# pigBond/olympics-mujoco

Hardware: AMD Instinct MI355X
Metric: env-steps/sec, 4096 UnitreeH1.walk envs per GPU, obs+reward+done+ctrl HIP kernel (higher is better)
Workload: dtype f64; 1 GPU; UnitreeH1.walk config-2: fused K1+K5 over one [T,N] block per step; T=400, envs_per_gpu=4096, launch_regime=[T,N] block per launch, io=qpos/qvel f64 + action f32 in; obs/reward/ctrl f32 + absorbing u8 out, parallelism=env-sharded x1, no data-path collective

## Files before the change

olympics-mujoco_amd/csrc/host_batcher.hip:

```cpp
#include <atomic>
#include <chrono>
#include <condition_variable>
#include <mutex>
#include <thread>
#include <vector>

#include "oly_common.h"

struct WorkerPool {
  std::vector<std::thread> threads;
  std::mutex mu;
  std::condition_variable cv_go;
  std::atomic<long> generation{0};
  std::atomic<int> pending{0};
  std::atomic<int> sleepers{0};
  std::atomic<bool> stop{false};
  static constexpr int kSpinUs = 200;

  static double now() {
    return std::chrono::duration<double>(std::chrono::steady_clock::now().time_since_epoch()).count();
  }
  static void relax() { __builtin_ia32_pause(); }

  template <class Job>
  void start(int n, Job job) {
    for (int id = 0; id < n; ++id)
      threads.emplace_back([this, job, id] {
        long seen = 0;
        for (;;) {
          const double t0 = now();
          int polls = 0;
          while (generation.load(std::memory_order_acquire) == seen && !stop.load(std::memory_order_acquire)) {
            relax();
            if ((++polls & 63) == 0 && (now() - t0) * 1e6 > kSpinUs) {
              std::unique_lock<std::mutex> lk(mu);
              sleepers.fetch_add(1);
              cv_go.wait(lk, [&] { return stop.load() || generation.load() != seen; });
              sleepers.fetch_sub(1);
            }
          }
          if (stop.load(std::memory_order_acquire)) return;
          seen = generation.load(std::memory_order_acquire);
          job(id);
          pending.fetch_sub(1, std::memory_order_release);
        }
      });
  }
  void run() {
    pending.store((int)threads.size(), std::memory_order_relaxed);
    generation.fetch_add(1);
    if (sleepers.load() > 0) {
      std::lock_guard<std::mutex> lk(mu);
      cv_go.notify_all();
    }
    int polls = 0;
    while (pending.load(std::memory_order_acquire) != 0) {
      relax();
      if ((++polls & 1023) == 0) std::this_thread::yield();
    }
  }
  void shutdown() {
    {
      std::lock_guard<std::mutex> lk(mu);
      stop.store(true, std::memory_order_release);
    }
    cv_go.notify_all();
    for (auto& t : threads) t.join();
    threads.clear();
  }
};

struct oly_batcher {
  oly_ctx* ctx;
  int N, nq, nv, nu, n_act, n_threads;
  double dt;
  oly_physics_fn fn;
  void* user;
  double *h_qpos, *h_qvel, *h_ctrl;
  double *d_qpos, *d_qvel, *d_ctrl, *d_prev;
  int mapped;
  double *m_qpos, *m_qvel, *m_ctrl;
  int W, C;
  oly_physics_contacts_fn cfn;
  void* cuser;
  unsigned char *h_con, *d_con;
  size_t con_bytes, off_g1, off_g2, off_f6;
  double* d_grf;
  uint8_t* d_over;
  std::atomic<int> overflow_env;
  int packed;
  double *h_grfw, *d_grfw;
  std::vector<std::vector<unsigned char>> scratch;
  WorkerPool pool;
  double timing[3];
};

namespace {

void kinematic_step(int, const double*, double* qpos, double* qvel, void* user) {
  const oly_batcher* b = static_cast<const oly_batcher*>(user);
  const int n = b->nq < b->nv ? b->nq : b->nv;
  for (int i = 0; i < n; ++i) qpos[i] += b->dt * qvel[i];
}

void pack_env(oly_batcher* b, int e, const oly_il_contacts& oc, double* out_base) {
  const oly_ctx* ctx = b->ctx;
  const int P = ctx->grf.n_pairs, K = 3 * P, C = b->C;
  for (int w = 0; w < b->W; ++w) {
    const int nc_raw = oc.ncon[(size_t)w * oc.ncon_stride];
    if (!out_base && nc_raw >= 0 && nc_raw <= C) continue;
    double* out = out_base ? out_base + ((size_t)w * b->N + e) * K : nullptr;
    if (out) for (int k = 0; k < K; ++k) out[k] = 0.0;
    const int nc = nc_raw < 0 ? 0 : (nc_raw > C ? C : nc_raw);
    const int32_t *g1 = oc.geom1 + (size_t)w * oc.geom_stride, *g2 = oc.geom2 + (size_t)w * oc.geom_stride;
    const double* f6 = oc.force6 + (size_t)w * oc.force_stride;
    bool over = nc_raw < 0;
    for (int p = 0; p < P; ++p) {
      bool found = false;
      for (int i = 0; i < nc; ++i) {
        const int a = g1[i], c2 = g2[i];
        const int ga = (a >= 0 && a < ctx->grf.ngeom) ? ctx->grf_group_host[a] : -1;
        const int gb = (c2 >= 0 && c2 < ctx->grf.ngeom) ? ctx->grf_group_host[c2] : -1;
        if (ga < 0 || gb < 0) continue;
        if ((ga == ctx->grf.pair_a[p] && gb == ctx->grf.pair_b[p]) || (ga == ctx->grf.pair_b[p] && gb == ctx->grf.pair_a[p])) {
          if (out) { const double* f = f6 + (size_t)i * 6; out[3 * p] = f[0]; out[3 * p + 1] = f[1]; out[3 * p + 2] = f[2]; }
          found = true;
          break;
        }
      }
      if (!found && nc_raw > C) over = true;
    }
    if (over) {
      int none = -1;
      b->overflow_env.compare_exchange_strong(none, e);
    }
  }
}

void run_range(oly_batcher* b, int lo, int hi, int id) {
  if (b->cfn && b->packed) {
    const size_t W = (size_t)b->W, C = (size_t)b->C;
    unsigned char* sc = b->scratch[id].data();
    int32_t* ncon = reinterpret_cast<int32_t*>(sc);
    const size_t off_g1 = (sizeof(int32_t) * W + 15) & ~(size_t)15;
    const size_t off_g2 = off_g1 + sizeof(int32_t) * W * C;
    const size_t off_f6 = (off_g2 + sizeof(int32_t) * W * C + 15) & ~(size_t)15;
    for (int e = lo; e < hi; ++e) {
      oly_il_contacts oc;
      oc.W = b->W; oc.C = b->C;
      oc.ncon = ncon; oc.ncon_stride = 1;
      oc.geom1 = reinterpret_cast<int32_t*>(sc + off_g1);
      oc.geom2 = reinterpret_cast<int32_t*>(sc + off_g2);
      oc.geom_stride = (long)C;
      oc.force6 = reinterpret_cast<double*>(sc + off_f6);
      oc.force_stride = (long)(C * 6);
      b->cfn(e, b->h_ctrl + (size_t)e * b->nu, b->h_qpos + (size_t)e * b->nq, b->h_qvel + (size_t)e * b->nv, &oc,
             b->cuser);
      pack_env(b, e, oc, b->h_grfw);
    }
    return;
  }
  if (b->cfn) {
    const size_t N = (size_t)b->N, C = (size_t)b->C;
    for (int e = lo; e < hi; ++e) {
      oly_il_contacts oc;
      oc.W = b->W; oc.C = b->C;
      oc.ncon = reinterpret_cast<int32_t*>(b->h_con) + e; oc.ncon_stride = (long)N;
      oc.geom1 = reinterpret_cast<int32_t*>(b->h_con + b->off_g1) + (size_t)e * C;
      oc.geom2 = reinterpret_cast<int32_t*>(b->h_con + b->off_g2) + (size_t)e * C;
      oc.geom_stride = (long)(N * C);
      oc.force6 = reinterpret_cast<double*>(b->h_con + b->off_f6) + (size_t)e * C * 6;
      oc.force_stride = (long)(N * C * 6);
      b->cfn(e, b->h_ctrl + (size_t)e * b->nu, b->h_qpos + (size_t)e * b->nq, b->h_qvel + (size_t)e * b->nv, &oc,
             b->cuser);
      pack_env(b, e, oc, nullptr);
    }
    return;
  }
  void* user = b->fn == kinematic_step ? static_cast<void*>(b) : b->user;
  for (int e = lo; e < hi; ++e)
    b->fn(e, b->h_ctrl + (size_t)e * b->nu, b->h_qpos + (size_t)e * b->nq, b->h_qvel + (size_t)e * b->nv, user);
}

void worker_main(oly_batcher* b, int id) {
  const int per = (b->N + b->n_threads - 1) / b->n_threads;
  const int lo = id * per, hi = lo + per < b->N ? lo + per : b->N;
  if (lo < hi) run_range(b, lo, hi, id);
}

double now_s() {
  return std::chrono::duration<double>(std::chrono::steady_clock::now().time_since_epoch()).count();
}

}

extern "C" int oly_batcher_create(oly_batcher** out, oly_ctx* ctx, int N, int n_threads, double dt,
                                  oly_physics_fn physics, void* user) {
  if (!out || !ctx) return OLY_EINVAL;
  *out = nullptr;
  if (!ctx->il_ok) OLY_FAIL(ctx, OLY_ENOTCONF, "oly_batcher_create before oly_il_configure");
  if (N <= 0 || n_threads < 0) OLY_FAIL(ctx, OLY_EINVAL, "oly_batcher_create: bad N or n_threads");
  OLY_HIP(ctx, hipSetDevice(ctx->device));
  oly_batcher* b = new (std::nothrow) oly_batcher();
  if (!b) return OLY_ENOMEM;
  const IlDev& h = ctx->il_host;
  b->ctx = ctx; b->N = N; b->nq = h.nq; b->nv = h.nv; b->nu = h.nu; b->n_act = h.n_act; b->dt = dt;
  b->fn = physics ? physics : kinematic_step;
  b->user = user;
  unsigned hw = std::thread::hardware_concurrency();
  if (n_threads == 0) n_threads = hw ? (int)hw : 1;
  if (n_threads > N) n_threads = N;
  b->n_threads = n_threads;
  b->h_qpos = b->h_qvel = b->h_ctrl = nullptr;
  b->d_qpos = b->d_qvel = b->d_ctrl = b->d_prev = nullptr;
  b->W = b->C = 0; b->cfn = nullptr; b->cuser = nullptr; b->h_con = b->d_con = nullptr; b->d_grf = nullptr;
  b->d_over = nullptr; b->overflow_env.store(-1);
  b->packed = 0; b->h_grfw = b->d_grfw = nullptr;
  b->mapped = 0; b->m_qpos = b->m_qvel = b->m_ctrl = nullptr;
  const size_t sq = sizeof(double) * N * b->nq, sv = sizeof(double) * N * b->nv, sc = sizeof(double) * N * b->nu;
  bool ok = hipHostMalloc(reinterpret_cast<void**>(&b->h_qpos), sq, hipHostMallocDefault) == hipSuccess &&
            hipHostMalloc(reinterpret_cast<void**>(&b->h_qvel), sv, hipHostMallocDefault) == hipSuccess &&
            hipHostMalloc(reinterpret_cast<void**>(&b->h_ctrl), sc, hipHostMallocDefault) == hipSuccess &&
            hipMalloc(reinterpret_cast<void**>(&b->d_qpos), sq) == hipSuccess &&
            hipMalloc(reinterpret_cast<void**>(&b->d_qvel), sv) == hipSuccess &&
            hipMalloc(reinterpret_cast<void**>(&b->d_ctrl), sc) == hipSuccess &&
            hipMalloc(reinterpret_cast<void**>(&b->d_prev), sizeof(double) * N) == hipSuccess;
  if (!ok) {
    oly_batcher_destroy(b);
    OLY_FAIL(ctx, OLY_ENOMEM, "oly_batcher_create: allocation failed (N=%d)", N);
  }
  memset(b->h_qpos, 0, sq); memset(b->h_qvel, 0, sv); memset(b->h_ctrl, 0, sc);
  (void)hipMemset(b->d_prev, 0, sizeof(double) * N);
  b->pool.start(n_threads, [b](int id) { worker_main(b, id); });
  *out = b;
  return OLY_OK;
}

extern "C" void oly_batcher_destroy(oly_batcher* b) {
  if (!b) return;
  b->pool.shutdown();
  if (b->h_qpos) (void)hipHostFree(b->h_qpos);
  if (b->h_qvel) (void)hipHostFree(b->h_qvel);
  if (b->h_ctrl) (void)hipHostFree(b->h_ctrl);
  if (b->d_qpos) (void)hipFree(b->d_qpos);
  if (b->d_qvel) (void)hipFree(b->d_qvel);
  if (b->d_ctrl) (void)hipFree(b->d_ctrl);
  if (b->d_prev) (void)hipFree(b->d_prev);
  if (b->h_con) (void)hipHostFree(b->h_con);
  if (b->d_con) (void)hipFree(b->d_con);
  if (b->d_grf) (void)hipFree(b->d_grf);
  if (b->d_over) (void)hipFree(b->d_over);
  if (b->h_grfw) (void)hipHostFree(b->h_grfw);
  if (b->d_grfw) (void)hipFree(b->d_grfw);
  delete b;
}

extern "C" int oly_batcher_enable_contacts(oly_batcher* b, int W, int C, oly_physics_contacts_fn physics, void* user) {
  if (!b) return OLY_EINVAL;
  oly_ctx* ctx = b->ctx;
  if (W <= 0 || C <= 0 || !physics) OLY_FAIL(ctx, OLY_EINVAL, "oly_batcher_enable_contacts: bad W, C or NULL physics");
  if (!ctx->grf_ok) OLY_FAIL(ctx, OLY_ENOTCONF, "oly_batcher_enable_contacts before oly_grf_configure");
  if (ctx->il_host.n_grf != 3 * ctx->grf.n_pairs)
    OLY_FAIL(ctx, OLY_EINVAL, "oly_batcher_enable_contacts: model n_grf=%d but %d sensor pairs", ctx->il_host.n_grf,
             ctx->grf.n_pairs);
  if (b->h_con) OLY_FAIL(ctx, OLY_EINVAL, "oly_batcher_enable_contacts: already enabled");
  OLY_HIP(ctx, hipSetDevice(ctx->device));
  const size_t N = (size_t)b->N;
  auto al = [](size_t x) { return (x + 15) & ~(size_t)15; };
  b->off_g1 = al(sizeof(int32_t) * W * N);
  b->off_g2 = al(b->off_g1 + sizeof(int32_t) * W * N * C);
  b->off_f6 = al(b->off_g2 + sizeof(int32_t) * W * N * C);
  b->con_bytes = al(b->off_f6 + sizeof(double) * W * N * C * 6);
  if (hipHostMalloc(reinterpret_cast<void**>(&b->h_con), b->con_bytes, hipHostMallocDefault) != hipSuccess ||
      hipMalloc(reinterpret_cast<void**>(&b->d_con), b->con_bytes) != hipSuccess ||
      hipMalloc(reinterpret_cast<void**>(&b->d_grf), sizeof(double) * N * ctx->il_host.n_grf) != hipSuccess ||
      hipMalloc(reinterpret_cast<void**>(&b->d_over), N) != hipSuccess)
    OLY_FAIL(ctx, OLY_ENOMEM, "oly_batcher_enable_contacts: allocation failed");
  memset(b->h_con, 0, b->con_bytes);
  b->W = W; b->C = C; b->cuser = user;
  b->cfn = physics;
  return OLY_OK;
}

extern "C" int oly_batcher_enable_contacts_packed(oly_batcher* b, int W, int C, oly_physics_contacts_fn physics,
                                                  void* user) {
  if (!b) return OLY_EINVAL;
  oly_ctx* ctx = b->ctx;
  if (W <= 0 || C <= 0 || !physics) OLY_FAIL(ctx, OLY_EINVAL, "oly_batcher_enable_contacts_packed: bad W, C or NULL physics");
  if (!ctx->grf_ok || !ctx->grf_group_host) OLY_FAIL(ctx, OLY_ENOTCONF, "oly_batcher_enable_contacts_packed before oly_grf_configure");
  if (ctx->il_host.n_grf != 3 * ctx->grf.n_pairs)
    OLY_FAIL(ctx, OLY_EINVAL, "oly_batcher_enable_contacts_packed: model n_grf=%d but %d sensor pairs", ctx->il_host.n_grf,
             ctx->grf.n_pairs);
  if (b->cfn) OLY_FAIL(ctx, OLY_EINVAL, "oly_batcher_enable_contacts_packed: contacts already enabled");
  OLY_HIP(ctx, hipSetDevice(ctx->device));
  const size_t N = (size_t)b->N, K = (size_t)ctx->il_host.n_grf;
  if (hipHostMalloc(reinterpret_cast<void**>(&b->h_grfw), sizeof(double) * W * N * K, hipHostMallocDefault) != hipSuccess ||
      hipMalloc(reinterpret_cast<void**>(&b->d_grfw), sizeof(double) * W * N * K) != hipSuccess ||
      hipMalloc(reinterpret_cast<void**>(&b->d_grf), sizeof(double) * N * K) != hipSuccess)
    OLY_FAIL(ctx, OLY_ENOMEM, "oly_batcher_enable_contacts_packed: allocation failed");
  const size_t slab = ((sizeof(int32_t) * W + 15) & ~(size_t)15) + 2 * sizeof(int32_t) * W * C + 16 + sizeof(double) * W * C * 6;
  b->scratch.assign((size_t)(b->n_threads > 0 ? b->n_threads : 1), std::vector<unsigned char>(slab, 0));
  b->W = W; b->C = C; b->cuser = user; b->packed = 1;
  b->cfn = physics;
  return OLY_OK;
}

extern "C" int oly_batcher_set_mapped(oly_batcher* b, int on) {
  if (!b) return OLY_EINVAL;
  oly_ctx* ctx = b->ctx;
  if (on && !b->m_qpos) {
    OLY_HIP(ctx, hipHostGetDevicePointer(reinterpret_cast<void**>(&b->m_qpos), b->h_qpos, 0));
    OLY_HIP(ctx, hipHostGetDevicePointer(reinterpret_cast<void**>(&b->m_qvel), b->h_qvel, 0));
    OLY_HIP(ctx, hipHostGetDevicePointer(reinterpret_cast<void**>(&b->m_ctrl), b->h_ctrl, 0));
  }
  b->mapped = on & 3;
  return OLY_OK;
}

extern "C" double* oly_batcher_qpos(oly_batcher* b) { return b ? b->h_qpos : nullptr; }
extern "C" double* oly_batcher_qvel(oly_batcher* b) { return b ? b->h_qvel : nullptr; }
extern "C" double* oly_batcher_prev(oly_batcher* b) { return b ? b->d_prev : nullptr; }

extern "C" int oly_batcher_set_prev(oly_batcher* b, const double* prev_dev, oly_stream stream) {
  if (!b || !prev_dev) return OLY_EINVAL;
  OLY_HIP(b->ctx, hipMemcpyAsync(b->d_prev, prev_dev, sizeof(double) * b->N, hipMemcpyDeviceToDevice, oly_s(stream)));
  return OLY_OK;
}

extern "C" int oly_batcher_last_timing(const oly_batcher* b, double out3[3]) {
  if (!b || !out3) return OLY_EINVAL;
  for (int i = 0; i < 3; ++i) out3[i] = b->timing[i];
  return OLY_OK;
}

extern "C" int oly_batcher_step(oly_batcher* b, const float* action, void* obs, float* reward,
                                uint8_t* absorbing, uint8_t* fall_code, int out_flags, oly_stream stream) {
  if (!b) return OLY_EINVAL;
  oly_ctx* ctx = b->ctx;
  if (!action || !obs || !reward || !absorbing) OLY_FAIL(ctx, OLY_EINVAL, "oly_batcher_step: NULL pointer");
  hipStream_t s = oly_s(stream);
  const double t0 = now_s();
  int rc = oly_il_ctrl(ctx, b->N, action, (b->mapped & 1) ? b->m_ctrl : b->d_ctrl, OLY_OUT_CTRL_F64, stream);
  if (rc) return rc;
  if (!(b->mapped & 1))
    OLY_HIP(ctx, hipMemcpyAsync(b->h_ctrl, b->d_ctrl, sizeof(double) * b->N * b->nu, hipMemcpyDeviceToHost, s));
  OLY_HIP(ctx, hipStreamSynchronize(s));
  const double t1 = now_s();
  b->overflow_env.store(-1);
  b->pool.run();
  const double t2 = now_s();
  const int oe = b->overflow_env.load();
  if (!(b->mapped & 2)) {
    OLY_HIP(ctx, hipMemcpyAsync(b->d_qpos, b->h_qpos, sizeof(double) * b->N * b->nq, hipMemcpyHostToDevice, s));
    OLY_HIP(ctx, hipMemcpyAsync(b->d_qvel, b->h_qvel, sizeof(double) * b->N * b->nv, hipMemcpyHostToDevice, s));
  }
  const double* grf = nullptr;
  if (b->cfn && b->packed) {
    const size_t K = (size_t)ctx->il_host.n_grf;
    OLY_HIP(ctx, hipMemcpyAsync(b->d_grfw, b->h_grfw, sizeof(double) * b->W * b->N * K, hipMemcpyHostToDevice, s));
    rc = oly_il_grf_window(ctx, b->W, b->N, (int)K, b->d_grfw, b->d_grf, stream);
    if (rc) return rc;
    grf = b->d_grf;
  } else if (b->cfn) {
    OLY_HIP(ctx, hipMemcpyAsync(b->d_con, b->h_con, b->con_bytes, hipMemcpyHostToDevice, s));
    rc = oly_il_ground_forces(ctx, b->W, b->N, b->C, reinterpret_cast<const int32_t*>(b->d_con),
                              reinterpret_cast<const int32_t*>(b->d_con + b->off_g1),
                              reinterpret_cast<const int32_t*>(b->d_con + b->off_g2),
                              reinterpret_cast<const double*>(b->d_con + b->off_f6), nullptr, b->d_grf, b->d_over, stream);
    if (rc) return rc;
    grf = b->d_grf;
  } else if (ctx->il_host.n_grf > 0) {
    OLY_FAIL(ctx, OLY_ENOTCONF, "oly_batcher_step: the model has foot-force columns; call oly_batcher_enable_contacts");
  }
  rc = oly_il_step(ctx, 1, b->N, (b->mapped & 2) ? b->m_qpos : b->d_qpos, (b->mapped & 2) ? b->m_qvel : b->d_qvel, nullptr, grf,
                   b->d_prev, b->d_prev, obs, reward,
                   absorbing, fall_code, nullptr, out_flags & ~OLY_OUT_CTRL_F64, stream);
  const double t3 = now_s();
  b->timing[0] = t1 - t0; b->timing[1] = t2 - t1; b->timing[2] = t3 - t2;
  if (rc == OLY_OK && oe >= 0)
    OLY_FAIL(ctx, OLY_ERANGE, "oly_batcher_step: environment %d has more contacts than the %d staged slots and a sensor pair "
             "without a contact among them (or a negative count): its foot-force columns of this step are not the "
             "reference's; the step itself was completed (host and device state agree); enable contacts with more slots",
             oe, b->C);
  return rc;
}

struct oly_a3_batcher {
  oly_ctx* ctx;
  int N, C, nq, nv, nu, n_threads;
  oly_a3_physics_fn fn;
  void* user;
  unsigned char *h_slab, *d_slab;
  size_t slab_bytes;
  size_t off[16];
  double *h_target, *d_target;
  double* m_target;
  int32_t *d_nr, *d_nl;
  double *d_grf_r, *d_grf_l, *d_minz;
  uint8_t* d_bad;
  int compact;
  unsigned char *hc_slab, *dc_slab;
  size_t coffs[16];
  size_t c_fixed_bytes, c_slab_bytes;
  std::vector<std::vector<oly_contact_record>> arena;
  std::vector<int> arena_count, arena_base;
  int* loc;
  int job_pack_only, job_phase;
  WorkerPool pool;
  double timing[3];
};

namespace {

enum { A_QPOS, A_QVEL, A_ALEN, A_AVEL, A_LFP, A_RFP, A_LFV, A_RFV, A_ROOTP, A_ROOTQ, A_HEAD, A_NCON, A_G1, A_G2, A_F6, A_CZ };

void a3_slots(const oly_a3_batcher* b, unsigned char* base, int e, oly_a3_readback* rb) {
  auto d = [&](int k, int w) { return reinterpret_cast<double*>(base + b->off[k]) + (size_t)e * w; };
  auto i = [&](int k, int w) { return reinterpret_cast<int32_t*>(base + b->off[k]) + (size_t)e * w; };
  rb->qpos = d(A_QPOS, b->nq); rb->qvel = d(A_QVEL, b->nv);
  rb->act_len = d(A_ALEN, b->nu); rb->act_vel = d(A_AVEL, b->nu);
  rb->lf_pos = d(A_LFP, 3); rb->rf_pos = d(A_RFP, 3); rb->lf_vel = d(A_LFV, 3); rb->rf_vel = d(A_RFV, 3);
  rb->root_pos = d(A_ROOTP, 3); rb->root_quat = d(A_ROOTQ, 4); rb->head_pos = d(A_HEAD, 3);
  rb->ncon = i(A_NCON, 1); rb->geom1 = i(A_G1, b->C); rb->geom2 = i(A_G2, b->C);
  rb->force6 = d(A_F6, 6 * b->C); rb->cpos_z = d(A_CZ, b->C);
}

void a3_hold_state(int, const double*, const oly_a3_readback*, void*) {}

enum { C_BQ, C_AV, C_ALEN, C_AVEL, C_LFP, C_RFP, C_LFV, C_RFV, C_ROOTP, C_ROOTQ, C_HEAD, C_NCON, C_COFF, C_REC };

template <class T>
T* c_ptr(const oly_a3_batcher* b, unsigned char* base, int k) { return reinterpret_cast<T*>(base + b->coffs[k]); }

void a3_pack_env(oly_a3_batcher* b, int id, int e, const oly_a3_readback& rb, int& cnt) {
  unsigned char* h = b->hc_slab;
  const int nu = b->nu;
  auto cp = [&](int k, const double* src, int w) { memcpy(c_ptr<double>(b, h, k) + (size_t)e * w, src, sizeof(double) * w); };
  cp(C_BQ, rb.qpos + 3, 4);
  cp(C_AV, rb.qvel + 3, 3);
  cp(C_ALEN, rb.act_len, nu); cp(C_AVEL, rb.act_vel, nu);
  cp(C_LFP, rb.lf_pos, 3); cp(C_RFP, rb.rf_pos, 3); cp(C_LFV, rb.lf_vel, 3); cp(C_RFV, rb.rf_vel, 3);
  cp(C_ROOTP, rb.root_pos, 3); cp(C_ROOTQ, rb.root_quat, 4); cp(C_HEAD, rb.head_pos, 3);
  const int nc_raw = rb.ncon[0];
  const int nc = nc_raw < 0 ? 0 : (nc_raw > b->C ? b->C : nc_raw);
  c_ptr<int32_t>(b, h, C_NCON)[e] = nc_raw;
  b->loc[e] = cnt;
  oly_contact_record* out = b->arena[id].data() + cnt;
  for (int i = 0; i < nc; ++i) {
    out[i].geom1 = rb.geom1[i];
    out[i].geom2 = rb.geom2[i];
    memcpy(out[i].force6, rb.force6 + 6 * i, sizeof(double) * 6);
    out[i].pos_z = rb.cpos_z[i];
  }
  cnt += nc;
}

void a3_worker(oly_a3_batcher* b, int id) {
  const int per = (b->N + b->n_threads - 1) / b->n_threads;
  const int lo = id * per, hi = lo + per < b->N ? lo + per : b->N;
  if (b->compact && b->job_phase == 1) {
    const int base = b->arena_base[id];
    memcpy(c_ptr<oly_contact_record>(b, b->hc_slab, C_REC) + base, b->arena[id].data(),
           sizeof(oly_contact_record) * (size_t)b->arena_count[id]);
    int32_t* coff = c_ptr<int32_t>(b, b->hc_slab, C_COFF);
    for (int e = lo; e < hi; ++e) coff[e] = base + b->loc[e];
    return;
  }
  int cnt = 0;
  for (int e = lo; e < hi; ++e) {
    oly_a3_readback rb;
    a3_slots(b, b->h_slab, e, &rb);
    if (!b->job_pack_only) b->fn(e, b->h_target + (size_t)e * b->nu, &rb, b->user);
    if (b->compact) a3_pack_env(b, id, e, rb, cnt);
  }
  if (b->compact) b->arena_count[id] = cnt;
}

}

extern "C" int oly_a3_batcher_create(oly_a3_batcher** out, oly_ctx* ctx, int N, int C, int n_threads,
                                     oly_a3_physics_fn physics, void* user) {
  if (!out || !ctx) return OLY_EINVAL;
  *out = nullptr;
  if (!ctx->a3_ok) OLY_FAIL(ctx, OLY_ENOTCONF, "oly_a3_batcher_create before oly_a3_configure");
  if (!ctx->contact_ok) OLY_FAIL(ctx, OLY_ENOTCONF, "oly_a3_batcher_create before oly_contact_configure");
  if (N <= 0 || C <= 0 || n_threads < 0)
    OLY_FAIL(ctx, OLY_EINVAL, "oly_a3_batcher_create: bad N, C or n_threads");
  OLY_HIP(ctx, hipSetDevice(ctx->device));
  oly_a3_batcher* b = new (std::nothrow) oly_a3_batcher();
  if (!b) return OLY_ENOMEM;
  const A3Dev& h = ctx->a3_host;
  b->ctx = ctx; b->N = N; b->C = C; b->nq = h.nq; b->nv = h.nv; b->nu = h.nu; b->user = user;
  b->fn = physics ? physics : a3_hold_state;
  unsigned hw = std::thread::hardware_concurrency();
  if (n_threads == 0) n_threads = hw ? (int)hw : 1;
  if (n_threads > N) n_threads = N;
  b->n_threads = n_threads;
  const size_t w8[11] = {(size_t)h.nq, (size_t)h.nv, (size_t)h.nu, (size_t)h.nu, 3, 3, 3, 3, 3, 4, 3};
  size_t o = 0;
  auto put = [&](int k, size_t bytes) { b->off[k] = o; o = (o + bytes + 15) & ~(size_t)15; };
  for (int k = 0; k < 11; ++k) put(k, sizeof(double) * N * w8[k]);
  put(A_NCON, sizeof(int32_t) * N);
  put(A_G1, sizeof(int32_t) * N * C);
  put(A_G2, sizeof(int32_t) * N * C);
  put(A_F6, sizeof(double) * N * C * 6);
  put(A_CZ, sizeof(double) * N * C);
  b->slab_bytes = o;
  b->h_slab = b->d_slab = nullptr; b->h_target = b->d_target = nullptr; b->m_target = nullptr;
  b->compact = 0; b->hc_slab = b->dc_slab = nullptr; b->loc = nullptr; b->job_pack_only = 0; b->job_phase = 0;
  b->d_nr = b->d_nl = nullptr; b->d_grf_r = b->d_grf_l = b->d_minz = nullptr; b->d_bad = nullptr;
  bool ok = hipHostMalloc(reinterpret_cast<void**>(&b->h_slab), o, hipHostMallocDefault) == hipSuccess &&
            hipMalloc(reinterpret_cast<void**>(&b->d_slab), o) == hipSuccess &&
            hipHostMalloc(reinterpret_cast<void**>(&b->h_target), sizeof(double) * N * h.nu, hipHostMallocDefault) == hipSuccess &&
            hipMalloc(reinterpret_cast<void**>(&b->d_target), sizeof(double) * N * h.nu) == hipSuccess &&
            hipMalloc(reinterpret_cast<void**>(&b->d_nr), sizeof(int32_t) * N) == hipSuccess &&
            hipMalloc(reinterpret_cast<void**>(&b->d_nl), sizeof(int32_t) * N) == hipSuccess &&
            hipMalloc(reinterpret_cast<void**>(&b->d_grf_r), sizeof(double) * N) == hipSuccess &&
            hipMalloc(reinterpret_cast<void**>(&b->d_grf_l), sizeof(double) * N) == hipSuccess &&
            hipMalloc(reinterpret_cast<void**>(&b->d_minz), sizeof(double) * N) == hipSuccess &&
            hipMalloc(reinterpret_cast<void**>(&b->d_bad), N) == hipSuccess;
  if (!ok) {
    oly_a3_batcher_destroy(b);
    OLY_FAIL(ctx, OLY_ENOMEM, "oly_a3_batcher_create: allocation failed (N=%d C=%d)", N, C);
  }
  memset(b->h_slab, 0, o);
  memset(b->h_target, 0, sizeof(double) * N * h.nu);
  b->pool.start(n_threads, [b](int id) { a3_worker(b, id); });
  *out = b;
  return OLY_OK;
}

extern "C" void oly_a3_batcher_destroy(oly_a3_batcher* b) {
  if (!b) return;
  b->pool.shutdown();
  if (b->h_slab) (void)hipHostFree(b->h_slab);
  if (b->d_slab) (void)hipFree(b->d_slab);
  if (b->h_target) (void)hipHostFree(b->h_target);
  if (b->d_target) (void)hipFree(b->d_target);
  if (b->hc_slab) (void)hipHostFree(b->hc_slab);
  if (b->dc_slab) (void)hipFree(b->dc_slab);
  free(b->loc);
  for (void* p : {(void*)b->d_nr, (void*)b->d_nl, (void*)b->d_grf_r, (void*)b->d_grf_l, (void*)b->d_minz, (void*)b->d_bad})
    if (p) (void)hipFree(p);
  delete b;
}

extern "C" int oly_a3_batcher_slots(oly_a3_batcher* b, int env, oly_a3_readback* rb) {
  if (!b || !rb || env < 0 || env >= b->N) return OLY_EINVAL;
  a3_slots(b, b->h_slab, env, rb);
  return OLY_OK;
}

extern "C" int oly_a3_batcher_upload(oly_a3_batcher* b, oly_stream stream) {
  if (!b) return OLY_EINVAL;
  OLY_HIP(b->ctx, hipMemcpyAsync(b->d_slab, b->h_slab, b->slab_bytes, hipMemcpyHostToDevice, oly_s(stream)));
  return OLY_OK;
}

extern "C" int oly_a3_batcher_set_compact(oly_a3_batcher* b, int on) {
  if (!b) return OLY_EINVAL;
  oly_ctx* ctx = b->ctx;
  if (on && !b->hc_slab) {
    const int N = b->N, nu = b->nu;
    const size_t w8[11] = {4, 3, (size_t)nu, (size_t)nu, 3, 3, 3, 3, 3, 4, 3};
    size_t o = 0;
    auto put = [&](int k, size_t bytes) { b->coffs[k] = o; o = (o + bytes + 15) & ~(size_t)15; };
    for (int k = 0; k < 11; ++k) put(k, sizeof(double) * N * w8[k]);
    put(C_NCON, sizeof(int32_t) * N);
    put(C_COFF, sizeof(int32_t) * N);
    b->c_fixed_bytes = o;
    put(C_REC, sizeof(oly_contact_record) * (size_t)N * b->C);
    b->c_slab_bytes = o;
    OLY_HIP(ctx, hipSetDevice(ctx->device));
    if (hipHostMalloc(reinterpret_cast<void**>(&b->hc_slab), o, hipHostMallocDefault) != hipSuccess ||
        hipMalloc(reinterpret_cast<void**>(&b->dc_slab), o) != hipSuccess ||
        !(b->loc = static_cast<int*>(malloc(sizeof(int) * N))))
      OLY_FAIL(ctx, OLY_ENOMEM, "oly_a3_batcher_set_compact: allocation failed");
    memset(b->hc_slab, 0, o);
    const int per = (N + b->n_threads - 1) / b->n_threads;
    b->arena.assign((size_t)b->n_threads, std::vector<oly_contact_record>((size_t)per * b->C));
    b->arena_count.assign((size_t)b->n_threads, 0);
    b->arena_base.assign((size_t)b->n_threads, 0);
  }
  b->compact = on ? 1 : 0;
  return OLY_OK;
}

extern "C" int oly_a3_batcher_set_mapped(oly_a3_batcher* b, int on) {
  if (!b) return OLY_EINVAL;
  b->m_target = nullptr;
  if (on & 1) OLY_HIP(b->ctx, hipHostGetDevicePointer(reinterpret_cast<void**>(&b->m_target), b->h_target, 0));
  return OLY_OK;
}

extern "C" int oly_a3_batcher_last_timing(const oly_a3_batcher* b, double out3[3]) {
  if (!b || !out3) return OLY_EINVAL;
  for (int i = 0; i < 3; ++i) out3[i] = b->timing[i];
  return OLY_OK;
}

extern "C" int oly_a3_batcher_step(oly_a3_batcher* b, const float* action, const oly_a3_state* st, void* obs,
                                   float* rew6, float* reward, uint8_t* done, int out_flags, int with_physics,
                                   oly_stream stream) {
  if (!b) return OLY_EINVAL;
  oly_ctx* ctx = b->ctx;
  if (!st || !obs || !rew6 || !reward || !done || (with_physics && !action))
    OLY_FAIL(ctx, OLY_EINVAL, "oly_a3_batcher_step: NULL pointer");
  hipStream_t s = oly_s(stream);
  const double t0 = now_s();
  double t1 = t0, t2 = t0;
  if (with_physics) {
    int rc = oly_a3_pd_target(ctx, b->N, action, b->m_target ? b->m_target : b->d_target, stream);
    if (rc) return rc;
    if (!b->m_target)
      OLY_HIP(ctx, hipMemcpyAsync(b->h_target, b->d_target, sizeof(double) * b->N * b->nu, hipMemcpyDeviceToHost, s));
    OLY_HIP(ctx, hipStreamSynchronize(s));
    t1 = now_s();
    b->job_pack_only = 0; b->job_phase = 0;
    b->pool.run();
    t2 = now_s();
  } else if (b->compact) {
    b->job_pack_only = 1; b->job_phase = 0;
    b->pool.run();
  }
  if (b->compact) {
    int total = 0;
    for (int i = 0; i < b->n_threads; ++i) { b->arena_base[i] = total; total += b->arena_count[i]; }
    b->job_phase = 1;
    b->pool.run();
    b->job_phase = 0;
    t2 = with_physics ? now_s() : t2;
    unsigned char* d = b->dc_slab;
    OLY_HIP(ctx, hipMemcpyAsync(d, b->hc_slab, b->c_fixed_bytes + sizeof(oly_contact_record) * (size_t)total,
                                hipMemcpyHostToDevice, s));
    int rc = oly_contact_reduce_csr(ctx, b->N, b->C, c_ptr<int32_t>(b, d, C_NCON), c_ptr<int32_t>(b, d, C_COFF),
                                    c_ptr<oly_contact_record>(b, d, C_REC), (int64_t)total, b->d_nr, b->d_nl, b->d_grf_r,
                                    b->d_grf_l,
                                    b->d_minz, b->d_bad, stream);
    if (rc) return rc;
    oly_a3_inputs in;
    in.qpos = c_ptr<double>(b, d, C_BQ); in.qvel = c_ptr<double>(b, d, C_AV);
    in.act_len = c_ptr<double>(b, d, C_ALEN); in.act_vel = c_ptr<double>(b, d, C_AVEL);
    in.lf_pos = c_ptr<double>(b, d, C_LFP); in.rf_pos = c_ptr<double>(b, d, C_RFP);
    in.lf_vel = c_ptr<double>(b, d, C_LFV); in.rf_vel = c_ptr<double>(b, d, C_RFV);
    in.root_pos = c_ptr<double>(b, d, C_ROOTP); in.root_quat = c_ptr<double>(b, d, C_ROOTQ);
    in.head_pos = c_ptr<double>(b, d, C_HEAD);
    in.grf_l = b->d_grf_l; in.grf_r = b->d_grf_r; in.min_z = b->d_minz; in.n_r = b->d_nr; in.n_l = b->d_nl;
    in.bad = b->d_bad;
    rc = oly_a3_step_strided(ctx, b->N, &in, st, obs, rew6, reward, done, out_flags, 1, stream);
    const double t3 = now_s();
    b->timing[0] = t1 - t0; b->timing[1] = t2 - t1; b->timing[2] = t3 - t2;
    return rc;
  }
  OLY_HIP(ctx, hipMemcpyAsync(b->d_slab, b->h_slab, b->slab_bytes, hipMemcpyHostToDevice, s));
  oly_a3_readback rb;
  a3_slots(b, b->d_slab, 0, &rb);
  int rc = oly_contact_reduce(ctx, b->N, b->C, rb.ncon, rb.geom1, rb.geom2, rb.force6, rb.cpos_z, b->d_nr, b->d_nl,
                              nullptr, nullptr, b->d_grf_r, b->d_grf_l, b->d_minz, b->d_bad, stream);
  if (rc) return rc;
  oly_a3_inputs in;
  in.qpos = rb.qpos; in.qvel = rb.qvel; in.act_len = rb.act_len; in.act_vel = rb.act_vel;
  in.lf_pos = rb.lf_pos; in.rf_pos = rb.rf_pos; in.lf_vel = rb.lf_vel; in.rf_vel = rb.rf_vel;
  in.root_pos = rb.root_pos; in.root_quat = rb.root_quat; in.head_pos = rb.head_pos;
  in.grf_l = b->d_grf_l; in.grf_r = b->d_grf_r; in.min_z = b->d_minz; in.n_r = b->d_nr; in.n_l = b->d_nl;
  in.bad = b->d_bad;
  rc = oly_a3_step(ctx, b->N, &in, st, obs, rew6, reward, done, out_flags, stream);
  const double t3 = now_s();
  b->timing[0] = t1 - t0; b->timing[1] = t2 - t1; b->timing[2] = t3 - t2;
  return rc;
}
```

olympics-mujoco_amd/csrc/k1_il_step.hip:

```cpp
#include <cstdlib>

#include "oly_common.h"

namespace {

constexpr int THREADS = 256;
typedef unsigned int u32x4 __attribute__((ext_vector_type(4)));

template <int NQ, int NV, int NGRF, int NACT, int NU, int NOBS>
struct StaticDims {
  static constexpr int nq = NQ, nv = NV, n_grf = NGRF, n_act = NACT, nu = NU, n_obs = NOBS;
  static constexpr bool is_static = true;
  static constexpr int n_obs_ct = NOBS;
  template <int ROWS, int TH>
  static constexpr int max_chunks() {
    return (ROWS * (NQ + NV + NGRF) / 2 + ROWS * NACT / 4 + TH - 1) / TH;
  }
  __device__ explicit StaticDims(const IlDev*) {}
};
struct DynDims {
  int nq, nv, n_grf, n_act, nu, n_obs;
  static constexpr bool is_static = false;
  static constexpr int n_obs_ct = 1;
  template <int ROWS, int TH>
  static constexpr int max_chunks() { return 1; }
  __device__ explicit DynDims(const IlDev* m)
      : nq(m->nq), nv(m->nv), n_grf(m->n_grf), n_act(m->n_act), nu(m->nu), n_obs(m->n_obs) {}
};

struct IlArgs {
  const IlDev* md;
  long R;
  int N;
  const double* qpos;
  const double* qvel;
  const float* action;
  const double* grf;
  const double* prev_in;
  double* prev_out;
  void* obs;
  float* reward;
  uint8_t* absorbing;
  uint8_t* fall_code;
  void* ctrl;
  int fast;
  long tile0;
};

template <int ROWS, class D>
struct Carve {
  int q, v, g, a, tab_off, tab_str, tab_csrc, tab_act, total;
  __host__ __device__ Carve(int nq, int nv, int n_grf, int n_act, int nu, int n_obs) {
    auto al = [](int x) { return (x + 15) & ~15; };
    q = 0;
    v = q + ROWS * nq * 8;
    g = v + ROWS * nv * 8;
    a = al(g + ROWS * n_grf * 8);
    tab_off = al(a + ROWS * n_act * 4);
    tab_str = al(tab_off + n_obs * 4);
    tab_csrc = al(tab_str + n_obs * 4);
    tab_act = al(tab_csrc + nu * 4);
    total = al(tab_act + 4 * nu * 8);
  }
};

#ifndef OLY_K1_NT
#define OLY_K1_NT 1
#endif
typedef float f32x4 __attribute__((ext_vector_type(4)));
typedef double f64x2 __attribute__((ext_vector_type(2)));
__device__ __forceinline__ u32x4 ld16(const u32x4* p) {
  return (OLY_K1_NT & 1) ? __builtin_nontemporal_load(p) : *p;
}
__device__ __forceinline__ void st16(f32x4* p, f32x4 v) {
  if (OLY_K1_NT & 2) __builtin_nontemporal_store(v, p); else *p = v;
}
__device__ __forceinline__ void st16(f64x2* p, f64x2 v) {
  if (OLY_K1_NT & 2) __builtin_nontemporal_store(v, p); else *p = v;
}

#ifndef OLY_K1_ABLATE
#define OLY_K1_ABLATE 0
#endif

constexpr int FAST_FALL = 8;

template <int ROWS, class D, bool OBS64, bool CTRL64>
__global__ __launch_bounds__(THREADS) void il_step_kernel(IlArgs p) {
  extern __shared__ __attribute__((aligned(16))) unsigned char lds[];
  const IlDev* __restrict__ md = p.md;
  const D d(md);
  const Carve<ROWS, D> cv(d.nq, d.nv, d.n_grf, d.n_act, d.nu, d.n_obs);
  const int tid = threadIdx.x;
  const int lane = tid & 63;
  const long row0 = (p.tile0 + blockIdx.x) * ROWS;
  const int rows = (p.R - row0 < ROWS) ? (int)(p.R - row0) : ROWS;
  const bool full = (rows == ROWS) && p.fast;

  double* sq = reinterpret_cast<double*>(lds + cv.q);
  double* sv = reinterpret_cast<double*>(lds + cv.v);
  double* sg = reinterpret_cast<double*>(lds + cv.g);
  float* sa = reinterpret_cast<float*>(lds + cv.a);
  int* t_off = reinterpret_cast<int*>(lds + cv.tab_off);
  int* t_str = reinterpret_cast<int*>(lds + cv.tab_str);
  int* t_cidx = reinterpret_cast<int*>(lds + cv.tab_csrc);
  double* t_act = reinterpret_cast<double*>(lds + cv.tab_act);

  auto col_off = [&](int sidx) -> int {
    if (sidx < d.nq) return sidx;
    if (sidx < d.nq + d.nv) return ROWS * d.nq + (sidx - d.nq);
    return ROWS * (d.nq + d.nv) + (sidx - d.nq - d.nv);
  };
  auto col_str = [&](int sidx) -> int {
    if (sidx < d.nq) return d.nq;
    if (sidx < d.nq + d.nv) return d.nv;
    return d.n_grf;
  };
  const int first_grf = d.n_obs - d.n_grf;

  const int cq = ROWS * d.nq / 2, cvv = ROWS * d.nv / 2, cg = ROWS * d.n_grf / 2;
  const int ca = p.action ? ROWS * d.n_act / 4 : 0;
  const int cd = cq + cvv + cg;
  const int total = (OLY_K1_ABLATE & 2) ? 0 : cd + ca;
  u32x4* ld = reinterpret_cast<u32x4*>(sq);
  u32x4* la = reinterpret_cast<u32x4*>(sa);
  constexpr int MAXC = D::template max_chunks<ROWS, THREADS>();
  u32x4 regs[MAXC];
  const bool reg_staged = D::is_static && full;
  if (reg_staged) {
    const u32x4* gq = reinterpret_cast<const u32x4*>(p.qpos + row0 * d.nq);
    const u32x4* gv = reinterpret_cast<const u32x4*>(p.qvel + row0 * d.nv);
    const u32x4* gg = reinterpret_cast<const u32x4*>(p.grf ? p.grf + row0 * d.n_grf : nullptr);
    const u32x4* ga = reinterpret_cast<const u32x4*>(p.action ? p.action + row0 * d.n_act : nullptr);
#pragma unroll
    for (int k = 0; k < MAXC; ++k) {
      const int g = tid + k * THREADS;
      if (g < total) {
        const u32x4* src = g < cq ? gq + g : (g < cq + cvv ? gv + (g - cq) : (g < cd ? gg + (g - cq - cvv) : ga + (g - cd)));
        regs[k] = *src;
      }
    }
  }

  for (int i = tid; i < d.n_obs; i += THREADS) {
    const int sidx = md->src[i];
    t_off[i] = col_off(sidx);
    t_str[i] = col_str(sidx);
  }
  for (int j = tid; j < d.nu; j += THREADS) {
    const int k = md->ctrl_src[j];
    t_cidx[j] = k;
    const int kk = k < 0 ? 0 : k;
    t_act[j] = md->act_mean[kk];
    t_act[d.nu + j] = md->act_delta[kk];
    t_act[2 * d.nu + j] = md->ctrl_lo[kk];
    t_act[3 * d.nu + j] = md->ctrl_hi[kk];
  }
  constexpr int OW = OBS64 ? 2 : 4;
  const bool fixed_cols = D::is_static && ((THREADS * OW) % d.n_obs == 0);
  int my_off[OW], my_str[OW];
  if (fixed_cols) {
    const int c0 = (tid * OW) % d.n_obs;
#pragma unroll
    for (int k = 0; k < OW; ++k) {
      const int sidx = md->src[c0 + k];
      my_off[k] = col_off(sidx);
      my_str[k] = col_str(sidx);
    }
  }
  const int nf = md->n_fall;
  int f_off[FAST_FALL], f_str[FAST_FALL];
  double f_lo[FAST_FALL], f_hi[FAST_FALL];
  bool f_grf[FAST_FALL];
#pragma unroll
  for (int k = 0; k < FAST_FALL; ++k) {
    const int kk = k < nf ? k : 0;
    const int sidx = md->fall_sidx[kk];
    f_off[k] = col_off(sidx);
    f_str[k] = col_str(sidx);
    f_lo[k] = md->fall_lo[kk];
    f_hi[k] = md->fall_hi[kk];
    f_grf[k] = d.n_grf > 0 && md->fall_idx[kk] >= first_grf;
  }
  const int rt = md->reward_type;
  const int rew_off = col_off(md->reward_sidx), rew_str = col_str(md->reward_sidx);
  const bool rew_grf = d.n_grf > 0 && md->reward_idx >= first_grf;
  const double tvel = md->target_velocity;
  const int use_abs = md->use_absorbing;
  const long gr = row0 + tid;
  double prev0 = 0.0;
  if (tid < rows && rt != OLY_REWARD_NONE && gr < p.N) prev0 = p.prev_in[gr];

  if (reg_staged) {
#pragma unroll
    for (int k = 0; k < MAXC; ++k) {
      const int g = tid + k * THREADS;
      if (g < total) {
        if (g < cd) ld[g] = regs[k];
        else la[g - cd] = regs[k];
      }
    }
  } else if (full) {
    const u32x4* gq = reinterpret_cast<const u32x4*>(p.qpos + row0 * d.nq);
    const u32x4* gv = reinterpret_cast<const u32x4*>(p.qvel + row0 * d.nv);
    const u32x4* gg = reinterpret_cast<const u32x4*>(p.grf ? p.grf + row0 * d.n_grf : nullptr);
    const u32x4* ga = reinterpret_cast<const u32x4*>(p.action ? p.action + row0 * d.n_act : nullptr);
#pragma unroll 8
    for (int g = tid; g < total; g += THREADS) {
      const u32x4* src = g < cq ? gq + g : (g < cq + cvv ? gv + (g - cq) : (g < cd ? gg + (g - cq - cvv) : ga + (g - cd)));
      const u32x4 x = *src;
      if (g < cd) ld[g] = x;
      else la[g - cd] = x;
    }
  } else {
    for (int i = tid; i < rows * d.nq; i += THREADS) sq[i] = p.qpos[row0 * d.nq + i];
    for (int i = tid; i < rows * d.nv; i += THREADS) sv[i] = p.qvel[row0 * d.nv + i];
    if (p.grf)
      for (int i = tid; i < rows * d.n_grf; i += THREADS) sg[i] = p.grf[row0 * d.n_grf + i];
    if (p.action)
      for (int i = tid; i < rows * d.n_act; i += THREADS) sa[i] = p.action[row0 * d.n_act + i];
  }
  __syncthreads();
  if (OLY_K1_ABLATE == 1) {
    if (sq[tid] == 1.2345e300) p.reward[0] = 1.f;
    return;
  }

  if (tid < ROWS && !(OLY_K1_ABLATE & 16)) {
    const int r = tid;
    unsigned code = 0, ab = 0;
    if (r < rows) {
      double fv[FAST_FALL];
#pragma unroll
      for (int k = 0; k < FAST_FALL; ++k)
        if (k < nf) fv[k] = sq[f_off[k] + r * f_str[k]];
#pragma unroll
      for (int k = 0; k < FAST_FALL; ++k)
        if (k < nf) {
          const double v = f_grf[k] ? fv[k] / 1000.0 : fv[k];
          if (code == 0 && (v < f_lo[k] || v > f_hi[k])) code = (unsigned)(k + 1);
        }
      for (int k = FAST_FALL; k < nf; ++k) {
        const int sidx = md->fall_sidx[k];
        double v = sq[col_off(sidx) + r * col_str(sidx)];
        if (d.n_grf > 0 && md->fall_idx[k] >= first_grf) v = v / 1000.0;
        if (code == 0 && (v < md->fall_lo[k] || v > md->fall_hi[k])) code = (unsigned)(k + 1);
      }
      ab = (code != 0 && use_abs) ? 1u : 0u;
      if (rt == OLY_REWARD_NONE) {
        p.reward[gr] = 0.0f;
      } else {
        double x = sq[rew_off + r * rew_str];
        if (rew_grf) x = x / 1000.0;
        auto f = [&](double s) -> float {
          if (rt == OLY_REWARD_TARGET_VELOCITY) {
            const double dv = s - tvel;
            return (float)exp(-(dv * dv));
          }
          return (float)s;
        };
        if (gr < p.N) p.reward[gr] = f(prev0);
        if (gr + p.N < p.R)
          p.reward[gr + p.N] = f(x);
        else
          p.prev_out[gr - (p.R - p.N)] = x;
      }
    }
    if (full) {
      unsigned a4 = 0, c4 = 0;
#pragma unroll
      for (int k = 0; k < 4; ++k) {
        const int srcl = (lane & 15) * 4 + k;
        a4 |= (unsigned)__shfl((int)ab, srcl, 64) << (8 * k);
        c4 |= (unsigned)__shfl((int)code, srcl, 64) << (8 * k);
      }
      if (lane < 16) {
        const long q4 = (row0 + (r - lane)) / 4 + lane;
        reinterpret_cast<unsigned*>(p.absorbing)[q4] = a4;
        if (p.fall_code) reinterpret_cast<unsigned*>(p.fall_code)[q4] = c4;
      }
    } else if (r < rows) {
      p.absorbing[row0 + r] = (uint8_t)ab;
      if (p.fall_code) p.fall_code[row0 + r] = (uint8_t)code;
    }
  }

  auto obs_val = [&](int r, int c) -> double {
    const double x = sq[t_off[c] + r * t_str[c]];
    if (d.n_grf > 0 && c >= first_grf) return x / 1000.0;
    return x;
  };

  if (full) {
    const int nvec = ROWS * d.n_obs / OW;
    if (fixed_cols) {
      const int c0 = (tid * OW) % d.n_obs;
      const int rstep = THREADS * OW / d.n_obs;
      constexpr int NIT = (ROWS * D::n_obs_ct / OW + THREADS - 1) / THREADS;
      double v[NIT > 0 ? NIT : 1][OW];
#pragma unroll
      for (int it = 0; it < NIT; ++it) {
        const int r = tid * OW / d.n_obs + it * rstep;
#pragma unroll
        for (int k = 0; k < OW; ++k) v[it][k] = (OLY_K1_ABLATE & 4) ? (double)(r + k) : sq[my_off[k] + r * my_str[k]];
      }
#pragma unroll
      for (int it = 0; it < NIT; ++it) {
        const int i = tid + it * THREADS;
        if (i < nvec) {
#pragma unroll
          for (int k = 0; k < OW; ++k)
            if (d.n_grf > 0 && c0 + k >= first_grf) v[it][k] = v[it][k] / 1000.0;
          if (OBS64) {
            double2 o;
            o.x = v[it][0]; o.y = v[it][OW - 1];
            reinterpret_cast<double2*>(static_cast<double*>(p.obs) + row0 * d.n_obs)[i] = o;
          } else {
            float4 o;
            o.x = (float)v[it][0]; o.y = (float)v[it][1 % OW];
            o.z = (float)v[it][2 % OW]; o.w = (float)v[it][3 % OW];
            reinterpret_cast<float4*>(static_cast<float*>(p.obs) + row0 * d.n_obs)[i] = o;
          }
        }
      }
    } else if (OBS64) {
      double2* out = reinterpret_cast<double2*>(static_cast<double*>(p.obs) + row0 * d.n_obs);
      for (int i = tid; i < nvec; i += THREADS) {
        int e = 2 * i, r = e / d.n_obs, c = e - r * d.n_obs;
        double2 o;
        o.x = obs_val(r, c);
        if (++c == d.n_obs) { c = 0; ++r; }
        o.y = obs_val(r, c);
        out[i] = o;
      }
    } else {
      float4* out = reinterpret_cast<float4*>(static_cast<float*>(p.obs) + row0 * d.n_obs);
      for (int i = tid; i < nvec; i += THREADS) {
        int e = 4 * i, r = e / d.n_obs, c = e - r * d.n_obs;
        float4 o;
        o.x = (float)obs_val(r, c);
        if (++c == d.n_obs) { c = 0; ++r; }
        o.y = (float)obs_val(r, c);
        if (++c == d.n_obs) { c = 0; ++r; }
        o.z = (float)obs_val(r, c);
        if (++c == d.n_obs) { c = 0; ++r; }
        o.w = (float)obs_val(r, c);
        out[i] = o;
      }
    }
  } else {
    for (int e = tid; e < rows * d.n_obs; e += THREADS) {
      const int r = e / d.n_obs, c = e - r * d.n_obs;
      const double v = obs_val(r, c);
      if (OBS64)
        static_cast<double*>(p.obs)[row0 * d.n_obs + e] = v;
      else
        static_cast<float*>(p.obs)[row0 * d.n_obs + e] = (float)v;
    }
  }

  if (p.ctrl) {
    auto ctrl_val = [&](int r, int j) -> double {
      if (OLY_K1_ABLATE & 8) return (double)(r - j);
      const int k = t_cidx[j];
      const double a = (double)sa[r * d.n_act + (k < 0 ? 0 : k)];
      double u = a * t_act[d.nu + j] + t_act[j];
      const double lo = t_act[2 * d.nu + j], hi = t_act[3 * d.nu + j];
      if (u < lo) u = lo;
      if (u > hi) u = hi;
      return k < 0 ? 0.0 : u;
    };
    if (full && !CTRL64) {
      float4* out = reinterpret_cast<float4*>(static_cast<float*>(p.ctrl) + row0 * d.nu);
      const int n4 = ROWS * d.nu / 4;
      for (int i = tid; i < n4; i += THREADS) {
        int e = 4 * i, r = e / d.nu, j = e - r * d.nu;
        float4 o;
        o.x = (float)ctrl_val(r, j);
        if (++j == d.nu) { j = 0; ++r; }
        o.y = (float)ctrl_val(r, j);
        if (++j == d.nu) { j = 0; ++r; }
        o.z = (float)ctrl_val(r, j);
        if (++j == d.nu) { j = 0; ++r; }
        o.w = (float)ctrl_val(r, j);
        out[i] = o;
      }
    } else {
      for (int e = tid; e < rows * d.nu; e += THREADS) {
        const int r = e / d.nu, j = e - r * d.nu;
        const double u = ctrl_val(r, j);
        if (CTRL64)
          static_cast<double*>(p.ctrl)[row0 * d.nu + e] = u;
        else
          static_cast<float*>(p.ctrl)[row0 * d.nu + e] = (float)u;
      }
    }
  }
}

template <int ROWS, class D, bool OBS64, bool CTRL64>
__global__ __launch_bounds__(THREADS) void il_tile_kernel(IlArgs p) {
  static_assert(D::is_static, "tile kernel needs compile-time dimensions");
  static_assert(ROWS % 64 == 0 && ROWS <= THREADS, "ROWS: whole waves, at most one row per lane");
  constexpr int NQ = D::nq, NV = D::nv, NG = D::n_grf, NA = D::n_act, NU = D::nu, NO = D::n_obs;
  constexpr int CQ = ROWS * NQ / 2, CV = ROWS * NV / 2, CG = ROWS * NG / 2, CA = ROWS * NA / 4;
  constexpr int KQ = (CQ + THREADS - 1) / THREADS, KV = (CV + THREADS - 1) / THREADS,
                KG = (CG + THREADS - 1) / THREADS, KA = (CA + THREADS - 1) / THREADS;
  constexpr int ND = NQ + NV + NG;
  constexpr int OW = OBS64 ? 2 : 4;
  static_assert((ROWS * NO) % OW == 0, "observation tile must split into whole lane vectors");
  constexpr int NOV = ROWS * NO / OW;
  constexpr int NIT = (NOV + THREADS - 1) / THREADS;
  constexpr int CW = CTRL64 ? 2 : 4;
  constexpr int NCV = ROWS * NU / CW;
  constexpr int NCI = (NCV + THREADS - 1) / THREADS;

  extern __shared__ __attribute__((aligned(16))) unsigned char lds[];
  double* sq = reinterpret_cast<double*>(lds);
  double* sv = sq + ROWS * NQ;
  double* sg = sv + ROWS * NV;
  float* sa = reinterpret_cast<float*>(lds + (size_t)ROWS * ND * 8);
  double* t_act = reinterpret_cast<double*>(lds + (size_t)ROWS * ND * 8 + (size_t)ROWS * NA * 4);
  const IlDev* __restrict__ md = p.md;
  const int tid = threadIdx.x, lane = tid & 63;
  const bool with_ctrl = p.ctrl != nullptr;

  auto col_off = [&](int sidx) -> int {
    return sidx < NQ ? sidx : sidx < NQ + NV ? ROWS * NQ + (sidx - NQ) : ROWS * (NQ + NV) + (sidx - NQ - NV);
  };
  auto col_str = [&](int sidx) -> int { return sidx < NQ ? NQ : sidx < NQ + NV ? NV : NG; };
  auto is_grf = [&](int sidx) -> bool { return NG > 0 && sidx >= NQ + NV; };

  for (int j = tid; j < NU; j += THREADS) {
    const int k = md->ctrl_src[j];
    const int kk = k < 0 ? 0 : k;
    t_act[j] = md->act_mean[kk];
    t_act[NU + j] = md->act_delta[kk];
    t_act[2 * NU + j] = md->ctrl_lo[kk];
    t_act[3 * NU + j] = md->ctrl_hi[kk];
  }
  int e_off[NIT][OW];
  unsigned e_grf = 0;
#pragma unroll
  for (int it = 0; it < NIT; ++it)
#pragma unroll
    for (int k = 0; k < OW; ++k) {
      const int e = (tid + it * THREADS) * OW + k;
      int off = 0;
      if (e < ROWS * NO) {
        const int r = e / NO, c = e - r * NO;
        const int sidx = md->src[c];
        off = col_off(sidx) + r * col_str(sidx);
        if (is_grf(sidx)) e_grf |= 1u << (it * OW + k);
      }
      e_off[it][k] = off;
    }
  static_assert(NIT * OW <= 32, "grf bitmask holds 32 values per lane");
  int c_aidx[NCI][CW];
  int c_j[NCI][CW];
#pragma unroll
  for (int it = 0; it < NCI; ++it)
#pragma unroll
    for (int q = 0; q < CW; ++q) {
      const int e = (tid + it * THREADS) * CW + q;
      const int r = e / NU, j = e - r * NU;
      int k = -1;
      if (e < ROWS * NU) k = md->ctrl_src[j];
      c_j[it][q] = j;
      c_aidx[it][q] = k < 0 ? -1 : r * NA + k;
    }
  const int nf = md->n_fall;
  int f_off[FAST_FALL], f_str[FAST_FALL];
  double f_lo[FAST_FALL], f_hi[FAST_FALL];
  unsigned f_grf = 0;
#pragma unroll
  for (int k = 0; k < FAST_FALL; ++k) {
    const int kk = k < nf ? k : 0;
    const int sidx = md->fall_sidx[kk];
    f_off[k] = col_off(sidx);
    f_str[k] = col_str(sidx);
    if (is_grf(sidx)) f_grf |= 1u << k;
    f_lo[k] = k < nf ? md->fall_lo[kk] : -__builtin_huge_val();
    f_hi[k] = k < nf ? md->fall_hi[kk] : __builtin_huge_val();
  }
  const int rt = md->reward_type;
  const int rew_off = col_off(md->reward_sidx), rew_str = col_str(md->reward_sidx);
  const bool rew_grf = is_grf(md->reward_sidx);
  const double tvel = md->target_velocity;
  const int use_abs = md->use_absorbing;
  auto rew_f = [&](double s) -> float {
    if (rt == OLY_REWARD_TARGET_VELOCITY) {
      const double dv = s - tvel;
      return (float)exp(-(dv * dv));
    }
    return (float)s;
  };

  const long ntiles = p.tile0;
  u32x4 rq[KQ], rv[KV], rg[KG > 0 ? KG : 1], ra[KA];
  auto issue_loads = [&](long t) {
    const long r0 = t * ROWS;
    const u32x4* gq = reinterpret_cast<const u32x4*>(p.qpos + r0 * NQ) + tid;
    const u32x4* gv = reinterpret_cast<const u32x4*>(p.qvel + r0 * NV) + tid;
#pragma unroll
    for (int k = 0; k < KQ; ++k)
      if (k * THREADS + THREADS <= CQ || tid + k * THREADS < CQ) rq[k] = ld16(gq + k * THREADS);
#pragma unroll
    for (int k = 0; k < KV; ++k)
      if (k * THREADS + THREADS <= CV || tid + k * THREADS < CV) rv[k] = ld16(gv + k * THREADS);
    if (NG > 0) {
      const u32x4* gg = reinterpret_cast<const u32x4*>(p.grf + r0 * NG) + tid;
#pragma unroll
      for (int k = 0; k < KG; ++k)
        if (k * THREADS + THREADS <= CG || tid + k * THREADS < CG) rg[k] = ld16(gg + k * THREADS);
    }
    if (with_ctrl) {
      const u32x4* ga = reinterpret_cast<const u32x4*>(p.action + r0 * NA) + tid;
#pragma unroll
      for (int k = 0; k < KA; ++k)
        if (k * THREADS + THREADS <= CA || tid + k * THREADS < CA) ra[k] = ld16(ga + k * THREADS);
    }
  };

  long tile = blockIdx.x;
  if (tile < ntiles) issue_loads(tile);
  for (; tile < ntiles; tile += gridDim.x) {
    const long row0 = tile * ROWS;
    {
      u32x4* lq = reinterpret_cast<u32x4*>(sq) + tid;
      u32x4* lv = reinterpret_cast<u32x4*>(sv) + tid;
      u32x4* la = reinterpret_cast<u32x4*>(sa) + tid;
#pragma unroll
      for (int k = 0; k < KQ; ++k)
        if (k * THREADS + THREADS <= CQ || tid + k * THREADS < CQ) lq[k * THREADS] = rq[k];
#pragma unroll
      for (int k = 0; k < KV; ++k)
        if (k * THREADS + THREADS <= CV || tid + k * THREADS < CV) lv[k * THREADS] = rv[k];
      if (NG > 0) {
        u32x4* lg = reinterpret_cast<u32x4*>(sg) + tid;
#pragma unroll
        for (int k = 0; k < KG; ++k)
          if (k * THREADS + THREADS <= CG || tid + k * THREADS < CG) lg[k * THREADS] = rg[k];
      }
      if (with_ctrl) {
#pragma unroll
        for (int k = 0; k < KA; ++k)
          if (k * THREADS + THREADS <= CA || tid + k * THREADS < CA) la[k * THREADS] = ra[k];
      }
    }
    __syncthreads();
    const long next = tile + gridDim.x;
    if (next < ntiles) issue_loads(next);

    if (tid < ROWS) {
      const int r = tid;
      const long gr = row0 + r;
      double fv[FAST_FALL];
#pragma unroll
      for (int k = 0; k < FAST_FALL; ++k) {
        fv[k] = sq[f_off[k] + r * f_str[k]];
        if (NG > 0 && ((f_grf >> k) & 1u)) fv[k] = fv[k] / 1000.0;
      }
      double x = sq[rew_off + r * rew_str];
      if (NG > 0 && rew_grf) x = x / 1000.0;
      unsigned code = 0;
#pragma unroll
      for (int k = FAST_FALL - 1; k >= 0; --k)
        if (fv[k] < f_lo[k] || fv[k] > f_hi[k]) code = (unsigned)(k + 1);
      const unsigned ab = (code != 0 && use_abs) ? 1u : 0u;
      if (rt == OLY_REWARD_NONE) {
        p.reward[gr] = 0.0f;
      } else {
        if (gr < p.N) p.reward[gr] = rew_f(p.prev_in[gr]);
        if (gr + p.N < p.R)
          p.reward[gr + p.N] = rew_f(x);
        else
          p.prev_out[gr - (p.R - p.N)] = x;
      }
      unsigned a4 = 0, c4 = 0;
#pragma unroll
      for (int k = 0; k < 4; ++k) {
        const int srcl = (lane & 15) * 4 + k;
        a4 |= (unsigned)__shfl((int)ab, srcl, 64) << (8 * k);
        c4 |= (unsigned)__shfl((int)code, srcl, 64) << (8 * k);
      }
      if (lane < 16) {
        const long q4 = (row0 + (r - lane)) / 4 + lane;
        reinterpret_cast<unsigned*>(p.absorbing)[q4] = a4;
        if (p.fall_code) reinterpret_cast<unsigned*>(p.fall_code)[q4] = c4;
      }
    }

    {
      double v[NIT][OW];
#pragma unroll
      for (int it = 0; it < NIT; ++it)
#pragma unroll
        for (int k = 0; k < OW; ++k) {
          v[it][k] = sq[e_off[it][k]];
          if (NG > 0 && ((e_grf >> (it * OW + k)) & 1u)) v[it][k] = v[it][k] / 1000.0;
        }
#pragma unroll
      for (int it = 0; it < NIT; ++it) {
        const int i = tid + it * THREADS;
        if (it * THREADS + THREADS <= NOV || i < NOV) {
          if (OBS64) {
            f64x2 o;
            o.x = v[it][0]; o.y = v[it][OW - 1];
            st16(reinterpret_cast<f64x2*>(static_cast<double*>(p.obs) + row0 * NO) + i, o);
          } else {
            f32x4 o;
            o.x = (float)v[it][0]; o.y = (float)v[it][1 % OW];
            o.z = (float)v[it][2 % OW]; o.w = (float)v[it][3 % OW];
            st16(reinterpret_cast<f32x4*>(static_cast<float*>(p.obs) + row0 * NO) + i, o);
          }
        }
      }
    }

    if (with_ctrl) {
#pragma unroll
      for (int it = 0; it < NCI; ++it) {
        const int i = tid + it * THREADS;
        if (it * THREADS + THREADS <= NCV || i < NCV) {
          double u[CW];
#pragma unroll
          for (int q = 0; q < CW; ++q) {
            const int ai = c_aidx[it][q], j = c_j[it][q];
            const double a = (double)sa[ai < 0 ? 0 : ai];
            double x = a * t_act[NU + j] + t_act[j];
            const double lo = t_act[2 * NU + j], hi = t_act[3 * NU + j];
            if (x < lo) x = lo;
            if (x > hi) x = hi;
            u[q] = ai < 0 ? 0.0 : x;
          }
          if (CTRL64) {
            f64x2 o;
            o.x = u[0]; o.y = u[CW - 1];
            st16(reinterpret_cast<f64x2*>(static_cast<double*>(p.ctrl) + row0 * NU) + i, o);
          } else {
            f32x4 o;
            o.x = (float)u[0]; o.y = (float)u[1 % CW]; o.z = (float)u[2 % CW]; o.w = (float)u[3 % CW];
            st16(reinterpret_cast<f32x4*>(static_cast<float*>(p.ctrl) + row0 * NU) + i, o);
          }
        }
      }
    }
    __syncthreads();
  }
}

template <bool CTRL64>
__global__ __launch_bounds__(THREADS) void il_ctrl_kernel(const IlDev* __restrict__ md, long total,
                                                          const float* __restrict__ action,
                                                          void* __restrict__ ctrl) {
  const int nu = md->nu, n_act = md->n_act;
  const long stride = (long)gridDim.x * THREADS;
  for (long e = (long)blockIdx.x * THREADS + threadIdx.x; e < total; e += stride) {
    const long r = e / nu;
    const int j = (int)(e - r * nu);
    const int k = md->ctrl_src[j];
    double u = 0.0;
    if (k >= 0) {
      u = (double)action[r * n_act + k] * md->act_delta[k] + md->act_mean[k];
      if (u < md->ctrl_lo[k]) u = md->ctrl_lo[k];
      if (u > md->ctrl_hi[k]) u = md->ctrl_hi[k];
    }
    if (CTRL64)
      static_cast<double*>(ctrl)[e] = u;
    else
      static_cast<float*>(ctrl)[e] = (float)u;
  }
}

constexpr int DYN_ROWS = 64;

struct DynCarve {
  int a, eo, co, tact, total;
  __host__ __device__ DynCarve(int nq, int nv, int n_grf, int n_act, int nu, int n_obs) {
    auto al = [](int x) { return (x + 15) & ~15; };
    a = al(DYN_ROWS * (nq + nv + n_grf) * 8);
    eo = al(a + DYN_ROWS * n_act * 4);
    co = al(eo + DYN_ROWS * n_obs * 4);
    tact = al(co + DYN_ROWS * nu * 4);
    total = al(tact + 4 * nu * 8);
  }
};

template <bool OBS64, bool CTRL64>
__global__ __launch_bounds__(THREADS) void il_dyn_tile_kernel(IlArgs p) {
  constexpr int ROWS = DYN_ROWS;
  extern __shared__ __attribute__((aligned(16))) unsigned char lds[];
  const IlDev* __restrict__ md = p.md;
  const int nq = md->nq, nv = md->nv, n_grf = md->n_grf, n_act = md->n_act, nu = md->nu, n_obs = md->n_obs;
  const DynCarve cv(nq, nv, n_grf, n_act, nu, n_obs);
  const int tid = threadIdx.x, lane = tid & 63;
  double* sq = reinterpret_cast<double*>(lds);
  float* sa = reinterpret_cast<float*>(lds + cv.a);
  unsigned* eo = reinterpret_cast<unsigned*>(lds + cv.eo);
  int* co = reinterpret_cast<int*>(lds + cv.co);
  double* t_act = reinterpret_cast<double*>(lds + cv.tact);
  const bool with_ctrl = p.ctrl != nullptr;
  const int first_grf = n_obs - n_grf;

  auto col_off = [&](int sidx) -> int {
    if (sidx < nq) return sidx;
    if (sidx < nq + nv) return ROWS * nq + (sidx - nq);
    return ROWS * (nq + nv) + (sidx - nq - nv);
  };
  auto col_str = [&](int sidx) -> int { return sidx < nq ? nq : (sidx < nq + nv ? nv : n_grf); };

  for (int e = tid; e < ROWS * n_obs; e += THREADS) {
    const int r = e / n_obs, c = e - r * n_obs;
    const int sidx = md->src[c];
    eo[e] = (unsigned)(col_off(sidx) + r * col_str(sidx)) | (c >= first_grf && n_grf > 0 ? 0x80000000u : 0u);
  }
  for (int e = tid; e < ROWS * nu; e += THREADS) {
    const int r = e / nu, j = e - r * nu;
    const int k = md->ctrl_src[j];
    co[e] = k < 0 ? -1 : (((r * n_act + k) << 8) | j);
  }
  for (int j = tid; j < nu; j += THREADS) {
    const int k = md->ctrl_src[j];
    const int kk = k < 0 ? 0 : k;
    t_act[j] = md->act_mean[kk];
    t_act[nu + j] = md->act_delta[kk];
    t_act[2 * nu + j] = md->ctrl_lo[kk];
    t_act[3 * nu + j] = md->ctrl_hi[kk];
  }
  const int nf = md->n_fall;
  const int rt = md->reward_type;
  const int rew_sidx = md->reward_sidx;
  const bool rew_grf = n_grf > 0 && md->reward_idx >= first_grf;
  const double tvel = md->target_velocity;
  const int use_abs = md->use_absorbing;
  auto rew_f = [&](double s) -> float {
    if (rt == OLY_REWARD_TARGET_VELOCITY) {
      const double dv = s - tvel;
      return (float)exp(-(dv * dv));
    }
    return (float)s;
  };

  const int cq = ROWS * nq / 2, cvv = ROWS * nv / 2, cg = ROWS * n_grf / 2;
  const int ca = with_ctrl ? ROWS * n_act / 4 : 0;
  constexpr int KQ = 5, KG = 1, KA = 3;
  u32x4 rq[KQ], rv[KQ], rg[KG], ra[KA];
  u32x4* lq = reinterpret_cast<u32x4*>(sq);
  u32x4* lv = lq + cq;
  u32x4* lg = lv + cvv;
  u32x4* la = reinterpret_cast<u32x4*>(sa);
  auto issue_loads = [&](long t) {
    const long r0 = t * ROWS;
    const u32x4* gq = reinterpret_cast<const u32x4*>(p.qpos + r0 * nq) + tid;
    const u32x4* gv = reinterpret_cast<const u32x4*>(p.qvel + r0 * nv) + tid;
#pragma unroll
    for (int k = 0; k < KQ; ++k)
      if (tid + k * THREADS < cq) rq[k] = ld16(gq + k * THREADS);
#pragma unroll
    for (int k = 0; k < KQ; ++k)
      if (tid + k * THREADS < cvv) rv[k] = ld16(gv + k * THREADS);
    if (cg > 0) {
      const u32x4* gg = reinterpret_cast<const u32x4*>(p.grf + r0 * n_grf) + tid;
#pragma unroll
      for (int k = 0; k < KG; ++k)
        if (tid + k * THREADS < cg) rg[k] = ld16(gg + k * THREADS);
    }
    if (ca > 0) {
      const u32x4* ga = reinterpret_cast<const u32x4*>(p.action + r0 * n_act) + tid;
#pragma unroll
      for (int k = 0; k < KA; ++k)
        if (tid + k * THREADS < ca) ra[k] = ld16(ga + k * THREADS);
    }
  };
  auto land = [&](long row0) {
#pragma unroll
    for (int k = 0; k < KQ; ++k)
      if (tid + k * THREADS < cq) lq[tid + k * THREADS] = rq[k];
#pragma unroll
    for (int k = 0; k < KQ; ++k)
      if (tid + k * THREADS < cvv) lv[tid + k * THREADS] = rv[k];
#pragma unroll
    for (int k = 0; k < KG; ++k)
      if (tid + k * THREADS < cg) lg[tid + k * THREADS] = rg[k];
#pragma unroll
    for (int k = 0; k < KA; ++k)
      if (tid + k * THREADS < ca) la[tid + k * THREADS] = ra[k];
    for (int g = tid + KQ * THREADS; g < cq; g += THREADS)
      lq[g] = ld16(reinterpret_cast<const u32x4*>(p.qpos + row0 * nq) + g);
    for (int g = tid + KQ * THREADS; g < cvv; g += THREADS)
      lv[g] = ld16(reinterpret_cast<const u32x4*>(p.qvel + row0 * nv) + g);
    for (int g = tid + KG * THREADS; g < cg; g += THREADS)
      lg[g] = ld16(reinterpret_cast<const u32x4*>(p.grf + row0 * n_grf) + g);
    for (int g = tid + KA * THREADS; g < ca; g += THREADS)
      la[g] = ld16(reinterpret_cast<const u32x4*>(p.action + row0 * n_act) + g);
  };

  const long ntiles = p.tile0;
  long tile = blockIdx.x;
  if (tile < ntiles) issue_loads(tile);
  __syncthreads();
  for (; tile < ntiles; tile += gridDim.x) {
    const long row0 = tile * ROWS;
    land(row0);
    __syncthreads();
    const long next = tile + gridDim.x;
    if (next < ntiles) issue_loads(next);

    if (tid < ROWS) {
      const int r = tid;
      const long gr = row0 + r;
      unsigned code = 0;
      for (int k = 0; k < nf; ++k) {
        const int sidx = md->fall_sidx[k];
        double v = sq[col_off(sidx) + r * col_str(sidx)];
        if (n_grf > 0 && md->fall_idx[k] >= first_grf) v = v / 1000.0;
        if (code == 0 && (v < md->fall_lo[k] || v > md->fall_hi[k])) code = (unsigned)(k + 1);
      }
      const unsigned ab = (code != 0 && use_abs) ? 1u : 0u;
      if (rt == OLY_REWARD_NONE) {
        p.reward[gr] = 0.0f;
      } else {
        double x = sq[col_off(rew_sidx) + r * col_str(rew_sidx)];
        if (rew_grf) x = x / 1000.0;
        if (gr < p.N) p.reward[gr] = rew_f(p.prev_in[gr]);
        if (gr + p.N < p.R)
          p.reward[gr + p.N] = rew_f(x);
        else
          p.prev_out[gr - (p.R - p.N)] = x;
      }
      unsigned a4 = 0, c4 = 0;
#pragma unroll
      for (int k = 0; k < 4; ++k) {
        const int srcl = (lane & 15) * 4 + k;
        a4 |= (unsigned)__shfl((int)ab, srcl, 64) << (8 * k);
        c4 |= (unsigned)__shfl((int)code, srcl, 64) << (8 * k);
      }
      if (lane < 16) {
        const long q4 = row0 / 4 + lane;
        reinterpret_cast<unsigned*>(p.absorbing)[q4] = a4;
        if (p.fall_code) reinterpret_cast<unsigned*>(p.fall_code)[q4] = c4;
      }
    }

    {
      constexpr int OW = OBS64 ? 2 : 4;
      const int nvec = ROWS * n_obs / OW;
#pragma unroll 2
      for (int i = tid; i < nvec; i += THREADS) {
        unsigned o4[OW];
        double v[OW];
#pragma unroll
        for (int k = 0; k < OW; ++k) o4[k] = eo[i * OW + k];
#pragma unroll
        for (int k = 0; k < OW; ++k) {
          v[k] = sq[o4[k] & 0x7fffffffu];
          if (o4[k] & 0x80000000u) v[k] = v[k] / 1000.0;
        }
        if (OBS64) {
          f64x2 o;
          o.x = v[0]; o.y = v[OW - 1];
          st16(reinterpret_cast<f64x2*>(static_cast<double*>(p.obs) + row0 * n_obs) + i, o);
        } else {
          f32x4 o;
          o.x = (float)v[0]; o.y = (float)v[1 % OW]; o.z = (float)v[2 % OW]; o.w = (float)v[3 % OW];
          st16(reinterpret_cast<f32x4*>(static_cast<float*>(p.obs) + row0 * n_obs) + i, o);
        }
      }
    }

    if (with_ctrl) {
      constexpr int CW = CTRL64 ? 2 : 4;
      const int ncv = ROWS * nu / CW;
      for (int i = tid; i < ncv; i += THREADS) {
        double u[CW];
#pragma unroll
        for (int q = 0; q < CW; ++q) {
          const int c = co[i * CW + q];
          const int j = c & 0xff, ai = c >> 8;
          const double a = (double)sa[c < 0 ? 0 : ai];
          double x = a * t_act[nu + (c < 0 ? 0 : j)] + t_act[c < 0 ? 0 : j];
          const double lo = t_act[2 * nu + (c < 0 ? 0 : j)], hi = t_act[3 * nu + (c < 0 ? 0 : j)];
          if (x < lo) x = lo;
          if (x > hi) x = hi;
          u[q] = c < 0 ? 0.0 : x;
        }
        if (CTRL64) {
          f64x2 o;
          o.x = u[0]; o.y = u[CW - 1];
          st16(reinterpret_cast<f64x2*>(static_cast<double*>(p.ctrl) + row0 * nu) + i, o);
        } else {
          f32x4 o;
          o.x = (float)u[0]; o.y = (float)u[1 % CW]; o.z = (float)u[2 % CW]; o.w = (float)u[3 % CW];
          st16(reinterpret_cast<f32x4*>(static_cast<float*>(p.ctrl) + row0 * nu) + i, o);
        }
      }
    }
    __syncthreads();
  }
}

using H1Dims = StaticDims<17, 17, 0, 11, 11, 32>;
using AtlasDims = StaticDims<16, 16, 0, 10, 10, 30>;
using TalosDims = StaticDims<18, 18, 0, 12, 12, 34>;
using H1FFDims = StaticDims<17, 17, 6, 11, 11, 38>;
using TalosFFDims = StaticDims<18, 18, 6, 12, 12, 40>;
using H1ArmsDims = StaticDims<25, 25, 0, 19, 19, 48>;
using H1ArmsNoBackDims = StaticDims<24, 24, 0, 18, 18, 46>;
using AtlasBackDims = StaticDims<19, 19, 0, 13, 13, 36>;
using ArmsNoBack28Dims = StaticDims<28, 28, 0, 22, 22, 54>;
using AtlasFullDims = StaticDims<31, 31, 0, 25, 25, 60>;
using TalosFullDims = StaticDims<30, 30, 0, 24, 24, 58>;

template <int ROWS, class D>
int launch_generic(oly_ctx* ctx, IlArgs a, long tile0, int out_flags, hipStream_t s) {
  const IlDev& h = ctx->il_host;
  Carve<ROWS, D> cv(h.nq, h.nv, h.n_grf, h.n_act, h.nu, h.n_obs);
  const long tiles = (a.R + ROWS - 1) / ROWS - tile0;
  if (tiles <= 0) return OLY_OK;
  if (tiles > 0x7fffffffL) OLY_FAIL(ctx, OLY_EINVAL, "oly_il_step: too many rows");
  a.tile0 = tile0;
  dim3 grid((unsigned)tiles), block(THREADS);
  const bool o64 = out_flags & OLY_OUT_OBS_F64, c64 = out_flags & OLY_OUT_CTRL_F64;
#define OLY_K1(O, C_)                                                                       \
  do {                                                                                      \
    auto k = il_step_kernel<ROWS, D, O, C_>;                                                \
    if (cv.total > 48 * 1024)                                                               \
      OLY_HIP(ctx, hipFuncSetAttribute(reinterpret_cast<const void*>(k),                    \
                                       hipFuncAttributeMaxDynamicSharedMemorySize, cv.total)); \
    hipLaunchKernelGGL(k, grid, block, cv.total, s, a);                                     \
  } while (0)
  if (o64 && c64) OLY_K1(true, true);
  else if (o64) OLY_K1(true, false);
  else if (c64) OLY_K1(false, true);
  else OLY_K1(false, false);
#undef OLY_K1
  OLY_LAUNCH_CHECK(ctx, "il_step_kernel");
  return OLY_OK;
}

template <int ROWS, class D>
int launch_fast(oly_ctx* ctx, IlArgs a, int out_flags, int wg_per_cu, hipStream_t s) {
  const long nfull = a.R / ROWS;
  if (nfull > 0) {
    const int lds = ROWS * (D::nq + D::nv + D::n_grf) * 8 + ROWS * D::n_act * 4 + 4 * D::nu * 8;
    int per_cu = (160 * 1024) / lds;
    if (per_cu > 8) per_cu = 8;
    if (wg_per_cu > 0) per_cu = wg_per_cu;
    long want = (long)ctx->num_cu * per_cu;
    if (want > nfull) want = nfull;
    IlArgs b = a;
    b.tile0 = nfull;
    dim3 grid((unsigned)want), block(THREADS);
    const bool o64 = out_flags & OLY_OUT_OBS_F64, c64 = out_flags & OLY_OUT_CTRL_F64;
#define OLY_K1T(O, C_)                                                                      \
  do {                                                                                      \
    auto k = il_tile_kernel<ROWS, D, O, C_>;                                                \
    if (lds > 48 * 1024)                                                                    \
      OLY_HIP(ctx, hipFuncSetAttribute(reinterpret_cast<const void*>(k),                    \
                                       hipFuncAttributeMaxDynamicSharedMemorySize, lds));   \
    hipLaunchKernelGGL(k, grid, block, lds, s, b);                                          \
  } while (0)
    if (o64 && c64) OLY_K1T(true, true);
    else if (o64) OLY_K1T(true, false);
    else if (c64) OLY_K1T(false, true);
    else OLY_K1T(false, false);
#undef OLY_K1T
    OLY_LAUNCH_CHECK(ctx, "il_tile_kernel");
  }
  if (nfull * ROWS < a.R) return launch_generic<ROWS, D>(ctx, a, nfull, out_flags, s);
  return OLY_OK;
}

int launch_dyn(oly_ctx* ctx, IlArgs a, int out_flags, hipStream_t s) {
  const IlDev& h = ctx->il_host;
  const DynCarve cv(h.nq, h.nv, h.n_grf, h.n_act, h.nu, h.n_obs);
  const long nfull = (a.fast && cv.total <= 150 * 1024) ? a.R / DYN_ROWS : 0;
  if (nfull > 0) {
    int per_cu = (160 * 1024) / cv.total;
    if (per_cu > 4) per_cu = 4;
    if (per_cu < 1) per_cu = 1;
    long want = (long)ctx->num_cu * per_cu;
    if (want > nfull) want = nfull;
    IlArgs b = a;
    b.tile0 = nfull;
    dim3 grid((unsigned)want), block(THREADS);
    const bool o64 = out_flags & OLY_OUT_OBS_F64, c64 = out_flags & OLY_OUT_CTRL_F64;
#define OLY_K1D(O, C_)                                                                      \
  do {                                                                                      \
    auto k = il_dyn_tile_kernel<O, C_>;                                                     \
    if (cv.total > 48 * 1024)                                                               \
      OLY_HIP(ctx, hipFuncSetAttribute(reinterpret_cast<const void*>(k),                    \
                                       hipFuncAttributeMaxDynamicSharedMemorySize, cv.total)); \
    hipLaunchKernelGGL(k, grid, block, cv.total, s, b);                                     \
  } while (0)
    if (o64 && c64) OLY_K1D(true, true);
    else if (o64) OLY_K1D(true, false);
    else if (c64) OLY_K1D(false, true);
    else OLY_K1D(false, false);
#undef OLY_K1D
    OLY_LAUNCH_CHECK(ctx, "il_dyn_tile_kernel");
  }
  if (nfull * DYN_ROWS < a.R) return launch_generic<DYN_ROWS, DynDims>(ctx, a, nfull, out_flags, s);
  return OLY_OK;
}

inline bool al16(const void* p) { return (reinterpret_cast<uintptr_t>(p) & 15) == 0; }

}

extern "C" int oly_il_configure(oly_ctx* ctx, const oly_il_model* m) {
  if (!ctx || !m) return OLY_EINVAL;
  const int n_spec = m->n_pos + m->n_vel;
  const int n_obs = n_spec - m->n_drop + m->n_grf;
  if (m->nq <= 0 || m->nv <= 0 || m->n_pos < 0 || m->n_vel < 0 || m->n_drop < 0 || m->n_grf < 0 ||
      m->n_drop > n_spec || n_obs <= 0 || n_obs > OLY_MAX_OBS || m->n_act < 0 ||
      m->n_act > OLY_MAX_ACT || m->nu < m->n_act || m->nu > OLY_MAX_ACT || m->n_fall < 0 ||
      m->n_fall > OLY_MAX_FALL)
    OLY_FAIL(ctx, OLY_EINVAL, "oly_il_configure: bad shape (n_obs=%d n_act=%d nu=%d n_fall=%d)",
             n_obs, m->n_act, m->nu, m->n_fall);
  if (!m->qpos_adr || !m->qvel_adr || (m->n_act && (!m->act_to_ctrl || !m->act_mean ||
      !m->act_delta || !m->ctrl_lo || !m->ctrl_hi)) || (m->n_fall && (!m->fall_idx || !m->fall_lo ||
      !m->fall_hi)))
    OLY_FAIL(ctx, OLY_EINVAL, "oly_il_configure: NULL table");
  ctx->il_ok = false;
  IlDev& h = ctx->il_host;
  memset(&h, 0, sizeof(h));
  h.nq = m->nq; h.nv = m->nv; h.n_pos = m->n_pos; h.n_vel = m->n_vel; h.n_drop = m->n_drop;
  h.n_grf = m->n_grf; h.n_act = m->n_act; h.nu = m->nu; h.n_obs = n_obs; h.n_fall = m->n_fall;
  h.reward_type = m->reward_type; h.reward_idx = m->reward_idx;
  h.use_absorbing = m->use_absorbing_states; h.target_velocity = m->target_velocity;
  if (h.reward_type < OLY_REWARD_NONE || h.reward_type > OLY_REWARD_X_POS)
    OLY_FAIL(ctx, OLY_EINVAL, "oly_il_configure: unknown reward_type %d", h.reward_type);
  if (h.reward_type != OLY_REWARD_NONE && (h.reward_idx < 0 || h.reward_idx >= n_obs))
    OLY_FAIL(ctx, OLY_ERANGE, "oly_il_configure: reward_idx %d outside [0,%d)", h.reward_idx, n_obs);
  for (int c = 0; c < n_obs; ++c) {
    const int slot = c + m->n_drop;
    int s;
    if (slot < m->n_pos) {
      s = m->qpos_adr[slot];
      if (s < 0 || s >= m->nq) OLY_FAIL(ctx, OLY_ERANGE, "qpos_adr[%d]=%d outside nq=%d", slot, s, m->nq);
    } else if (slot < n_spec) {
      s = m->qvel_adr[slot - m->n_pos];
      if (s < 0 || s >= m->nv) OLY_FAIL(ctx, OLY_ERANGE, "qvel_adr[%d]=%d outside nv=%d", slot - m->n_pos, s, m->nv);
      s += m->nq;
    } else {
      s = m->nq + m->nv + (slot - n_spec);
    }
    h.src[c] = (short)s;
  }
  for (int k = 0; k < m->n_fall; ++k) {
    if (m->fall_idx[k] < 0 || m->fall_idx[k] >= n_obs)
      OLY_FAIL(ctx, OLY_ERANGE, "fall_idx[%d]=%d outside [0,%d)", k, m->fall_idx[k], n_obs);
    h.fall_idx[k] = m->fall_idx[k]; h.fall_lo[k] = m->fall_lo[k]; h.fall_hi[k] = m->fall_hi[k];
    h.fall_sidx[k] = h.src[m->fall_idx[k]];
  }
  h.reward_sidx = (h.reward_type != OLY_REWARD_NONE) ? h.src[h.reward_idx] : 0;
  for (int j = 0; j < m->nu; ++j) h.ctrl_src[j] = -1;
  for (int k = 0; k < m->n_act; ++k) {
    const int j = m->act_to_ctrl[k];
    if (j < 0 || j >= m->nu) OLY_FAIL(ctx, OLY_ERANGE, "act_to_ctrl[%d]=%d outside nu=%d", k, j, m->nu);
    h.ctrl_src[j] = (short)k;
    h.act_mean[k] = m->act_mean[k]; h.act_delta[k] = m->act_delta[k];
    h.ctrl_lo[k] = m->ctrl_lo[k]; h.ctrl_hi[k] = m->ctrl_hi[k];
  }
  OLY_HIP(ctx, hipSetDevice(ctx->device));
  OLY_HIP(ctx, hipMemcpy(ctx->il_dev, &h, sizeof(h), hipMemcpyHostToDevice));
  ctx->il_ok = true;
  return OLY_OK;
}

extern "C" int oly_il_obs_dim(const oly_ctx* ctx) {
  if (!ctx || !ctx->il_ok) return OLY_ENOTCONF;
  return ctx->il_host.n_obs;
}

extern "C" int oly_il_step(oly_ctx* ctx, int T, int N, const double* qpos, const double* qvel,
                           const float* action, const double* grf_mean, const double* prev_in,
                           double* prev_out, void* obs, float* reward, uint8_t* absorbing,
                           uint8_t* fall_code, void* ctrl, int out_flags, oly_stream stream) {
  if (!ctx) return OLY_EINVAL;
  if (!ctx->il_ok) OLY_FAIL(ctx, OLY_ENOTCONF, "oly_il_step before oly_il_configure");
  const IlDev& h = ctx->il_host;
  if (T < 0 || N < 0) OLY_FAIL(ctx, OLY_EINVAL, "oly_il_step: negative T or N");
  if (T == 0 || N == 0) return OLY_OK;
  if (!qpos || !qvel || !obs || !reward || !absorbing)
    OLY_FAIL(ctx, OLY_EINVAL, "oly_il_step: NULL required pointer");
  if (h.reward_type != OLY_REWARD_NONE && (!prev_in || !prev_out))
    OLY_FAIL(ctx, OLY_EINVAL, "oly_il_step: prev_in/prev_out required by the reward");
  if (T > 1 && prev_in == prev_out && prev_in)
    OLY_FAIL(ctx, OLY_EINVAL, "oly_il_step: prev_in must not alias prev_out when T > 1");
  if (h.n_grf > 0 && !grf_mean) OLY_FAIL(ctx, OLY_EINVAL, "oly_il_step: grf_mean required (n_grf=%d)", h.n_grf);
  if (ctrl && !action) OLY_FAIL(ctx, OLY_EINVAL, "oly_il_step: ctrl requested without action");
  IlArgs a;
  a.md = ctx->il_dev; a.R = (long)T * N; a.N = N; a.qpos = qpos; a.qvel = qvel; a.action = action;
  a.grf = h.n_grf ? grf_mean : nullptr; a.prev_in = prev_in; a.prev_out = prev_out; a.obs = obs;
  a.reward = reward; a.absorbing = absorbing; a.fall_code = fall_code; a.ctrl = ctrl;
  a.fast = al16(qpos) && al16(qvel) && al16(action) && al16(grf_mean) && al16(obs) && al16(ctrl) &&
           ((reinterpret_cast<uintptr_t>(absorbing) & 3) == 0) &&
           ((reinterpret_cast<uintptr_t>(fall_code) & 3) == 0);
  a.tile0 = 0;
  auto shape = [&](int nq, int na, int no, int ng = 0) {
    return h.nq == nq && h.nv == nq && h.n_grf == ng && h.n_act == na && h.nu == na && h.n_obs == no &&
           h.n_pos == nq && h.n_vel == nq && h.n_drop == 2;
  };
  const bool fast_ok = a.fast && h.n_fall <= FAST_FALL;
  static const int wg_env = [] { const char* e = getenv("OLY_K1_WG_PER_CU"); return e ? atoi(e) : 0; }();
  static const int rows_env = [] { const char* e = getenv("OLY_K1_ROWS"); return e ? atoi(e) : 0; }();
#define OLY_K1_FAST(DIMS, DEFROWS)                                                              \
  do {                                                                                          \
    const int rows = rows_env ? rows_env : DEFROWS;                                             \
    if (rows == 64) return launch_fast<64, DIMS>(ctx, a, out_flags, wg_env, oly_s(stream));     \
    return launch_fast<128, DIMS>(ctx, a, out_flags, wg_env, oly_s(stream));                    \
  } while (0)
  if (fast_ok && shape(17, 11, 32)) OLY_K1_FAST(H1Dims, 128);
  if (fast_ok && shape(16, 10, 30)) OLY_K1_FAST(AtlasDims, 128);
  if (fast_ok && shape(18, 12, 34)) OLY_K1_FAST(TalosDims, 128);
  if (fast_ok && shape(17, 11, 38, 6)) OLY_K1_FAST(H1FFDims, 128);
  if (fast_ok && shape(18, 12, 40, 6)) OLY_K1_FAST(TalosFFDims, 128);
  if (fast_ok && shape(25, 19, 48)) OLY_K1_FAST(H1ArmsDims, 128);
  if (fast_ok && shape(24, 18, 46)) return launch_fast<128, H1ArmsNoBackDims>(ctx, a, out_flags, wg_env, oly_s(stream));
  if (fast_ok && shape(19, 13, 36)) return launch_fast<128, AtlasBackDims>(ctx, a, out_flags, wg_env, oly_s(stream));
  if (fast_ok && shape(28, 22, 54)) return launch_fast<128, ArmsNoBack28Dims>(ctx, a, out_flags, wg_env, oly_s(stream));
  if (fast_ok && shape(31, 25, 60)) return launch_fast<128, AtlasFullDims>(ctx, a, out_flags, wg_env, oly_s(stream));
  if (fast_ok && shape(30, 24, 58)) return launch_fast<128, TalosFullDims>(ctx, a, out_flags, wg_env, oly_s(stream));
#undef OLY_K1_FAST
  static const int dyn_env = [] { const char* e = getenv("OLY_K1_DYN_TILE"); return e ? atoi(e) : 1; }();
  if (dyn_env) return launch_dyn(ctx, a, out_flags, oly_s(stream));
  return launch_generic<64, DynDims>(ctx, a, 0, out_flags, oly_s(stream));
}

extern "C" int oly_il_ctrl(oly_ctx* ctx, int N, const float* action, void* ctrl, int out_flags,
                           oly_stream stream) {
  if (!ctx) return OLY_EINVAL;
  if (!ctx->il_ok) OLY_FAIL(ctx, OLY_ENOTCONF, "oly_il_ctrl before oly_il_configure");
  if (N < 0 || (N > 0 && (!action || !ctrl))) OLY_FAIL(ctx, OLY_EINVAL, "oly_il_ctrl: bad argument");
  if (N == 0) return OLY_OK;
  const long total = (long)N * ctx->il_host.nu;
  long nb = (total + THREADS - 1) / THREADS;
  if (nb > 4096) nb = 4096;
  if (out_flags & OLY_OUT_CTRL_F64)
    hipLaunchKernelGGL(il_ctrl_kernel<true>, dim3((unsigned)nb), dim3(THREADS), 0, oly_s(stream), ctx->il_dev,
                       total, action, ctrl);
  else
    hipLaunchKernelGGL(il_ctrl_kernel<false>, dim3((unsigned)nb), dim3(THREADS), 0, oly_s(stream), ctx->il_dev,
                       total, action, ctrl);
  OLY_LAUNCH_CHECK(ctx, "il_ctrl_kernel");
  return OLY_OK;
}
```

olympics-mujoco_amd/csrc/oly_common.h:

```cpp
#pragma once

#include <hip/hip_runtime.h>

#include <cstdint>
#include <cstdio>
#include <cstring>

#include "../../include/olympic_hip.h"


struct IlDev {
  int nq, nv, n_pos, n_vel, n_drop, n_grf, n_act, nu, n_obs, n_fall;
  int reward_type, reward_idx, use_absorbing, reward_sidx;
  double target_velocity;
  short src[OLY_MAX_OBS];
  int fall_idx[OLY_MAX_FALL], fall_sidx[OLY_MAX_FALL];
  double fall_lo[OLY_MAX_FALL], fall_hi[OLY_MAX_FALL];
  short ctrl_src[OLY_MAX_ACT];
  double act_mean[OLY_MAX_ACT], act_delta[OLY_MAX_ACT], ctrl_lo[OLY_MAX_ACT], ctrl_hi[OLY_MAX_ACT];
};

struct A3Dev {
  int nq, nv, nu, period, delay_frames, n_obs, pad0, pad1;
  double target_radius, mass, goal_height_ref, goal_speed_ref;
  double clock_lut[4 * OLY_MAX_PERIOD];
  double motor_offset[16], gear[16];
};

struct ContactDev {
  int ngeom, floor_body, rfoot_body, lfoot_body;
  int* geom_bodyid;
};

struct GrfDev {
  int ngeom, n_pairs;
  int pair_a[OLY_MAX_GRF_PAIRS], pair_b[OLY_MAX_GRF_PAIRS];
  int* geom_group;
};

struct TrajDev {
  int n_keys, n_traj, len, pad;
  double* rows;
};

#define OLY_STATS_MAX_BLOCKS 1024

struct oly_ctx {
  int device;
  char err[512];
  IlDev* il_dev;
  IlDev il_host;
  bool il_ok;
  A3Dev* a3_dev;
  A3Dev a3_host;
  bool a3_ok;
  ContactDev contact;
  bool contact_ok;
  TrajDev traj;
  bool traj_ok;
  GrfDev grf;
  bool grf_ok;
  int* grf_group_host;
  double* stats_ws;
  size_t stats_ws_bytes;
  bool mlp_attr_done = false;
  bool disc_attr_done = false;
  bool roll_attr_done = false;
  unsigned upd_attr_done = 0;
  unsigned scan_attr_done = 0;
  unsigned ilmlp_attr_done = 0;
  unsigned discfit_attr_done = 0;
  unsigned gail_attr_done = 0;
  int num_cu;
};

#define OLY_FAIL(ctx, code, ...)                                \
  do {                                                          \
    if (ctx) snprintf((ctx)->err, sizeof((ctx)->err), __VA_ARGS__); \
    return (code);                                              \
  } while (0)

#define OLY_HIP(ctx, expr)                                                             \
  do {                                                                                 \
    hipError_t e__ = (expr);                                                           \
    if (e__ != hipSuccess)                                                             \
      OLY_FAIL(ctx, OLY_EHIP, "%s failed: %s (%s:%d)", #expr, hipGetErrorString(e__), \
               __FILE__, __LINE__);                                                    \
  } while (0)

#define OLY_LAUNCH_CHECK(ctx, what)                                                           \
  do {                                                                                        \
    hipError_t e__ = hipGetLastError();                                                       \
    if (e__ != hipSuccess)                                                                    \
      OLY_FAIL(ctx, OLY_EHIP, "launch of %s failed: %s", what, hipGetErrorString(e__));       \
  } while (0)

int oly_stats_finish(oly_ctx* ctx, int nblocks, int64_t n, double* stats3_out, oly_stream stream);
int oly_a3_step_strided(oly_ctx* ctx, int N, const oly_a3_inputs* in, const oly_a3_state* st, void* obs, float* rew6,
                        float* reward, uint8_t* done, int out_flags, int compact_base, oly_stream stream);

static inline hipStream_t oly_s(oly_stream s) { return reinterpret_cast<hipStream_t>(s); }

__device__ __forceinline__ double wave_sum(double v) {
#pragma unroll
  for (int off = 32; off > 0; off >>= 1) v += __shfl_down(v, off, 64);
  return v;
}
```

Measured before the change: 12.41 billion env-steps/s.

## Fold ragged tail into tile kernel and add small-row launches for small batches

Turns the per-tile body into a device function so the persistent tile kernel can handle the ragged tail tile in an extra workgroup, which removes the second launch. For small R it adds a small-rows path (16/32/64 rows with a matching thread count) so more workgroups fill the CUs. Action-table gathers move to a host-precomputed act_tab, and the prev_in load is prefetched alongside the other inputs. The workload is T*N = 1.6M rows, so the small-row path is probably not taken, and the main effect comes from the fused tail and the lighter prologue.

```diff
diff --git a/olympics-mujoco_amd/csrc/host_batcher.hip b/olympics-mujoco_amd/csrc/host_batcher.hip
--- a/olympics-mujoco_amd/csrc/host_batcher.hip
+++ b/olympics-mujoco_amd/csrc/host_batcher.hip
@@ -372,9 +372,11 @@
   } else if (ctx->il_host.n_grf > 0) {
     OLY_FAIL(ctx, OLY_ENOTCONF, "oly_batcher_step: the model has foot-force columns; call oly_batcher_enable_contacts");
   }
+  ctx->il_max_wg = (b->mapped & 2) ? 128 : 0;
   rc = oly_il_step(ctx, 1, b->N, (b->mapped & 2) ? b->m_qpos : b->d_qpos, (b->mapped & 2) ? b->m_qvel : b->d_qvel, nullptr, grf,
                    b->d_prev, b->d_prev, obs, reward,
                    absorbing, fall_code, nullptr, out_flags & ~OLY_OUT_CTRL_F64, stream);
+  ctx->il_max_wg = 0;
   const double t3 = now_s();
   b->timing[0] = t1 - t0; b->timing[1] = t2 - t1; b->timing[2] = t3 - t2;
   if (rc == OLY_OK && oe >= 0)
diff --git a/olympics-mujoco_amd/csrc/k1_il_step.hip b/olympics-mujoco_amd/csrc/k1_il_step.hip
--- a/olympics-mujoco_amd/csrc/k1_il_step.hip
+++ b/olympics-mujoco_amd/csrc/k1_il_step.hip
@@ -45,6 +45,7 @@
   void* ctrl;
   int fast;
   long tile0;
+  int tile_wgs;
 };
 
 template <int ROWS, class D>
@@ -85,15 +86,15 @@
 
 constexpr int FAST_FALL = 8;
 
-template <int ROWS, class D, bool OBS64, bool CTRL64>
-__global__ __launch_bounds__(THREADS) void il_step_kernel(IlArgs p) {
+template <int ROWS, int TH, class D, bool OBS64, bool CTRL64>
+__device__ __forceinline__ void il_step_tile(const IlArgs& p, const long tile) {
   extern __shared__ __attribute__((aligned(16))) unsigned char lds[];
   const IlDev* __restrict__ md = p.md;
   const D d(md);
   const Carve<ROWS, D> cv(d.nq, d.nv, d.n_grf, d.n_act, d.nu, d.n_obs);
   const int tid = threadIdx.x;
   const int lane = tid & 63;
-  const long row0 = (p.tile0 + blockIdx.x) * ROWS;
+  const long row0 = tile * ROWS;
   const int rows = (p.R - row0 < ROWS) ? (int)(p.R - row0) : ROWS;
   const bool full = (rows == ROWS) && p.fast;
 
@@ -124,7 +125,7 @@
   const int total = (OLY_K1_ABLATE & 2) ? 0 : cd + ca;
   u32x4* ld = reinterpret_cast<u32x4*>(sq);
   u32x4* la = reinterpret_cast<u32x4*>(sa);
-  constexpr int MAXC = D::template max_chunks<ROWS, THREADS>();
+  constexpr int MAXC = D::template max_chunks<ROWS, TH>();
   u32x4 regs[MAXC];
   const bool reg_staged = D::is_static && full;
   if (reg_staged) {
@@ -134,7 +135,7 @@
     const u32x4* ga = reinterpret_cast<const u32x4*>(p.action ? p.action + row0 * d.n_act : nullptr);
 #pragma unroll
     for (int k = 0; k < MAXC; ++k) {
-      const int g = tid + k * THREADS;
+      const int g = tid + k * TH;
       if (g < total) {
         const u32x4* src = g < cq ? gq + g : (g < cq + cvv ? gv + (g - cq) : (g < cd ? gg + (g - cq - cvv) : ga + (g - cd)));
         regs[k] = *src;
@@ -142,22 +143,24 @@
     }
   }
 
-  for (int i = tid; i < d.n_obs; i += THREADS) {
+  const long gr = row0 + tid;
+  double prev0 = 0.0;
+  if (p.prev_in && tid < rows && gr < p.N) prev0 = p.prev_in[gr];
+
+  for (int i = tid; i < d.n_obs; i += TH) {
     const int sidx = md->src[i];
     t_off[i] = col_off(sidx);
     t_str[i] = col_str(sidx);
   }
-  for (int j = tid; j < d.nu; j += THREADS) {
-    const int k = md->ctrl_src[j];
-    t_cidx[j] = k;
-    const int kk = k < 0 ? 0 : k;
-    t_act[j] = md->act_mean[kk];
-    t_act[d.nu + j] = md->act_delta[kk];
-    t_act[2 * d.nu + j] = md->ctrl_lo[kk];
-    t_act[3 * d.nu + j] = md->ctrl_hi[kk];
+  for (int j = tid; j < d.nu; j += TH) {
+    t_cidx[j] = md->ctrl_src[j];
+    t_act[j] = md->act_tab[j];
+    t_act[d.nu + j] = md->act_tab[OLY_MAX_ACT + j];
+    t_act[2 * d.nu + j] = md->act_tab[2 * OLY_MAX_ACT + j];
+    t_act[3 * d.nu + j] = md->act_tab[3 * OLY_MAX_ACT + j];
   }
   constexpr int OW = OBS64 ? 2 : 4;
-  const bool fixed_cols = D::is_static && ((THREADS * OW) % d.n_obs == 0);
+  const bool fixed_cols = D::is_static && ((TH * OW) % d.n_obs == 0);
   int my_off[OW], my_str[OW];
   if (fixed_cols) {
     const int c0 = (tid * OW) % d.n_obs;
@@ -172,29 +175,25 @@
   int f_off[FAST_FALL], f_str[FAST_FALL];
   double f_lo[FAST_FALL], f_hi[FAST_FALL];
   bool f_grf[FAST_FALL];
+  static_assert(FAST_FALL <= OLY_MAX_FALL, "slot k is read whether or not the model uses it");
 #pragma unroll
   for (int k = 0; k < FAST_FALL; ++k) {
-    const int kk = k < nf ? k : 0;
-    const int sidx = md->fall_sidx[kk];
+    const int sidx = md->fall_sidx[k];
     f_off[k] = col_off(sidx);
     f_str[k] = col_str(sidx);
-    f_lo[k] = md->fall_lo[kk];
-    f_hi[k] = md->fall_hi[kk];
-    f_grf[k] = d.n_grf > 0 && md->fall_idx[kk] >= first_grf;
+    f_lo[k] = md->fall_lo[k];
+    f_hi[k] = md->fall_hi[k];
+    f_grf[k] = d.n_grf > 0 && md->fall_idx[k] >= first_grf;
   }
   const int rt = md->reward_type;
   const int rew_off = col_off(md->reward_sidx), rew_str = col_str(md->reward_sidx);
   const bool rew_grf = d.n_grf > 0 && md->reward_idx >= first_grf;
   const double tvel = md->target_velocity;
   const int use_abs = md->use_absorbing;
-  const long gr = row0 + tid;
-  double prev0 = 0.0;
-  if (tid < rows && rt != OLY_REWARD_NONE && gr < p.N) prev0 = p.prev_in[gr];
-
   if (reg_staged) {
 #pragma unroll
     for (int k = 0; k < MAXC; ++k) {
-      const int g = tid + k * THREADS;
+      const int g = tid + k * TH;
       if (g < total) {
         if (g < cd) ld[g] = regs[k];
         else la[g - cd] = regs[k];
@@ -206,19 +205,19 @@
     const u32x4* gg = reinterpret_cast<const u32x4*>(p.grf ? p.grf + row0 * d.n_grf : nullptr);
     const u32x4* ga = reinterpret_cast<const u32x4*>(p.action ? p.action + row0 * d.n_act : nullptr);
 #pragma unroll 8
-    for (int g = tid; g < total; g += THREADS) {
+    for (int g = tid; g < total; g += TH) {
       const u32x4* src = g < cq ? gq + g : (g < cq + cvv ? gv + (g - cq) : (g < cd ? gg + (g - cq - cvv) : ga + (g - cd)));
       const u32x4 x = *src;
       if (g < cd) ld[g] = x;
       else la[g - cd] = x;
     }
   } else {
-    for (int i = tid; i < rows * d.nq; i += THREADS) sq[i] = p.qpos[row0 * d.nq + i];
-    for (int i = tid; i < rows * d.nv; i += THREADS) sv[i] = p.qvel[row0 * d.nv + i];
+    for (int i = tid; i < rows * d.nq; i += TH) sq[i] = p.qpos[row0 * d.nq + i];
+    for (int i = tid; i < rows * d.nv; i += TH) sv[i] = p.qvel[row0 * d.nv + i];
     if (p.grf)
-      for (int i = tid; i < rows * d.n_grf; i += THREADS) sg[i] = p.grf[row0 * d.n_grf + i];
+      for (int i = tid; i < rows * d.n_grf; i += TH) sg[i] = p.grf[row0 * d.n_grf + i];
     if (p.action)
-      for (int i = tid; i < rows * d.n_act; i += THREADS) sa[i] = p.action[row0 * d.n_act + i];
+      for (int i = tid; i < rows * d.n_act; i += TH) sa[i] = p.action[row0 * d.n_act + i];
   }
   __syncthreads();
   if (OLY_K1_ABLATE == 1) {
@@ -226,7 +225,9 @@
     return;
   }
 
-  if (tid < ROWS && !(OLY_K1_ABLATE & 16)) {
+  static_assert(ROWS % 4 == 0 && ROWS <= TH && TH % 64 == 0, "ROWS: flags leave as dwords, at most one row per lane");
+  constexpr int RW = (ROWS + 63) / 64 * 64;
+  if (tid < RW && !(OLY_K1_ABLATE & 16)) {
     const int r = tid;
     unsigned code = 0, ab = 0;
     if (r < rows) {
@@ -274,7 +275,7 @@
         a4 |= (unsigned)__shfl((int)ab, srcl, 64) << (8 * k);
         c4 |= (unsigned)__shfl((int)code, srcl, 64) << (8 * k);
       }
-      if (lane < 16) {
+      if (lane < 16 && (r - lane) + 4 * lane < ROWS) {
         const long q4 = (row0 + (r - lane)) / 4 + lane;
         reinterpret_cast<unsigned*>(p.absorbing)[q4] = a4;
         if (p.fall_code) reinterpret_cast<unsigned*>(p.fall_code)[q4] = c4;
@@ -295,8 +296,8 @@
     const int nvec = ROWS * d.n_obs / OW;
     if (fixed_cols) {
       const int c0 = (tid * OW) % d.n_obs;
-      const int rstep = THREADS * OW / d.n_obs;
-      constexpr int NIT = (ROWS * D::n_obs_ct / OW + THREADS - 1) / THREADS;
+      const int rstep = TH * OW / d.n_obs;
+      constexpr int NIT = (ROWS * D::n_obs_ct / OW + TH - 1) / TH;
       double v[NIT > 0 ? NIT : 1][OW];
 #pragma unroll
       for (int it = 0; it < NIT; ++it) {
@@ -306,7 +307,7 @@
       }
 #pragma unroll
       for (int it = 0; it < NIT; ++it) {
-        const int i = tid + it * THREADS;
+        const int i = tid + it * TH;
         if (i < nvec) {
 #pragma unroll
           for (int k = 0; k < OW; ++k)
@@ -325,7 +326,7 @@
       }
     } else if (OBS64) {
       double2* out = reinterpret_cast<double2*>(static_cast<double*>(p.obs) + row0 * d.n_obs);
-      for (int i = tid; i < nvec; i += THREADS) {
+      for (int i = tid; i < nvec; i += TH) {
         int e = 2 * i, r = e / d.n_obs, c = e - r * d.n_obs;
         double2 o;
         o.x = obs_val(r, c);
@@ -335,7 +336,7 @@
       }
     } else {
       float4* out = reinterpret_cast<float4*>(static_cast<float*>(p.obs) + row0 * d.n_obs);
-      for (int i = tid; i < nvec; i += THREADS) {
+      for (int i = tid; i < nvec; i += TH) {
         int e = 4 * i, r = e / d.n_obs, c = e - r * d.n_obs;
         float4 o;
         o.x = (float)obs_val(r, c);
@@ -349,7 +350,7 @@
       }
     }
   } else {
-    for (int e = tid; e < rows * d.n_obs; e += THREADS) {
+    for (int e = tid; e < rows * d.n_obs; e += TH) {
       const int r = e / d.n_obs, c = e - r * d.n_obs;
       const double v = obs_val(r, c);
       if (OBS64)
@@ -373,7 +374,7 @@
     if (full && !CTRL64) {
       float4* out = reinterpret_cast<float4*>(static_cast<float*>(p.ctrl) + row0 * d.nu);
       const int n4 = ROWS * d.nu / 4;
-      for (int i = tid; i < n4; i += THREADS) {
+      for (int i = tid; i < n4; i += TH) {
         int e = 4 * i, r = e / d.nu, j = e - r * d.nu;
         float4 o;
         o.x = (float)ctrl_val(r, j);
@@ -386,7 +387,7 @@
         out[i] = o;
       }
     } else {
-      for (int e = tid; e < rows * d.nu; e += THREADS) {
+      for (int e = tid; e < rows * d.nu; e += TH) {
         const int r = e / d.nu, j = e - r * d.nu;
         const double u = ctrl_val(r, j);
         if (CTRL64)
@@ -396,6 +397,11 @@
       }
     }
   }
+}
+
+template <int ROWS, int TH, class D, bool OBS64, bool CTRL64>
+__global__ __launch_bounds__(TH) void il_step_kernel(IlArgs p) {
+  il_step_tile<ROWS, TH, D, OBS64, CTRL64>(p, p.tile0 + blockIdx.x);
 }
 
 template <int ROWS, class D, bool OBS64, bool CTRL64>
@@ -431,13 +437,47 @@
   auto col_str = [&](int sidx) -> int { return sidx < NQ ? NQ : sidx < NQ + NV ? NV : NG; };
   auto is_grf = [&](int sidx) -> bool { return NG > 0 && sidx >= NQ + NV; };
 
+  const long ntiles = p.tile0;
+  if ((int)blockIdx.x >= p.tile_wgs) {
+    il_step_tile<ROWS, THREADS, D, OBS64, CTRL64>(p, ntiles);
+    return;
+  }
+  const int wgs = p.tile_wgs;
+  u32x4 rq[KQ], rv[KV], rg[KG > 0 ? KG : 1], ra[KA];
+  double prev = 0.0;
+  auto issue_loads = [&](long t) {
+    const long r0 = t * ROWS;
+    const u32x4* gq = reinterpret_cast<const u32x4*>(p.qpos + r0 * NQ) + tid;
+    const u32x4* gv = reinterpret_cast<const u32x4*>(p.qvel + r0 * NV) + tid;
+#pragma unroll
+    for (int k = 0; k < KQ; ++k)
+      if (k * THREADS + THREADS <= CQ || tid + k * THREADS < CQ) rq[k] = ld16(gq + k * THREADS);
+#pragma unroll
+    for (int k = 0; k < KV; ++k)
+      if (k * THREADS + THREADS <= CV || tid + k * THREADS < CV) rv[k] = ld16(gv + k * THREADS);
+    if (NG > 0) {
+      const u32x4* gg = reinterpret_cast<const u32x4*>(p.grf + r0 * NG) + tid;
+#pragma unroll
+      for (int k = 0; k < KG; ++k)
+        if (k * THREADS + THREADS <= CG || tid + k * THREADS < CG) rg[k] = ld16(gg + k * THREADS);
+    }
+    if (with_ctrl) {
+      const u32x4* ga = reinterpret_cast<const u32x4*>(p.action + r0 * NA) + tid;
+#pragma unroll
+      for (int k = 0; k < KA; ++k)
+        if (k * THREADS + THREADS <= CA || tid + k * THREADS < CA) ra[k] = ld16(ga + k * THREADS);
+    }
+    if (p.prev_in && tid < ROWS && r0 + tid < p.N) prev = p.prev_in[r0 + tid];
+  };
+
+  long tile = blockIdx.x;
+  if (tile < ntiles) issue_loads(tile);
+
   for (int j = tid; j < NU; j += THREADS) {
-    const int k = md->ctrl_src[j];
-    const int kk = k < 0 ? 0 : k;
-    t_act[j] = md->act_mean[kk];
-    t_act[NU + j] = md->act_delta[kk];
-    t_act[2 * NU + j] = md->ctrl_lo[kk];
-    t_act[3 * NU + j] = md->ctrl_hi[kk];
+    t_act[j] = md->act_tab[j];
+    t_act[NU + j] = md->act_tab[OLY_MAX_ACT + j];
+    t_act[2 * NU + j] = md->act_tab[2 * OLY_MAX_ACT + j];
+    t_act[3 * NU + j] = md->act_tab[3 * OLY_MAX_ACT + j];
   }
   int e_off[NIT][OW];
   unsigned e_grf = 0;
@@ -475,13 +515,13 @@
   unsigned f_grf = 0;
 #pragma unroll
   for (int k = 0; k < FAST_FALL; ++k) {
-    const int kk = k < nf ? k : 0;
-    const int sidx = md->fall_sidx[kk];
+    const int sidx = md->fall_sidx[k];
+    const double lo = md->fall_lo[k], hi = md->fall_hi[k];
     f_off[k] = col_off(sidx);
     f_str[k] = col_str(sidx);
     if (is_grf(sidx)) f_grf |= 1u << k;
-    f_lo[k] = k < nf ? md->fall_lo[kk] : -__builtin_huge_val();
-    f_hi[k] = k < nf ? md->fall_hi[kk] : __builtin_huge_val();
+    f_lo[k] = k < nf ? lo : -__builtin_huge_val();
+    f_hi[k] = k < nf ? hi : __builtin_huge_val();
   }
   const int rt = md->reward_type;
   const int rew_off = col_off(md->reward_sidx), rew_str = col_str(md->reward_sidx);
@@ -496,35 +536,7 @@
     return (float)s;
   };
 
-  const long ntiles = p.tile0;
-  u32x4 rq[KQ], rv[KV], rg[KG > 0 ? KG : 1], ra[KA];
-  auto issue_loads = [&](long t) {
-    const long r0 = t * ROWS;
-    const u32x4* gq = reinterpret_cast<const u32x4*>(p.qpos + r0 * NQ) + tid;
-    const u32x4* gv = reinterpret_cast<const u32x4*>(p.qvel + r0 * NV) + tid;
-#pragma unroll
-    for (int k = 0; k < KQ; ++k)
-      if (k * THREADS + THREADS <= CQ || tid + k * THREADS < CQ) rq[k] = ld16(gq + k * THREADS);
-#pragma unroll
-    for (int k = 0; k < KV; ++k)
-      if (k * THREADS + THREADS <= CV || tid + k * THREADS < CV) rv[k] = ld16(gv + k * THREADS);
-    if (NG > 0) {
-      const u32x4* gg = reinterpret_cast<const u32x4*>(p.grf + r0 * NG) + tid;
-#pragma unroll
-      for (int k = 0; k < KG; ++k)
-        if (k * THREADS + THREADS <= CG || tid + k * THREADS < CG) rg[k] = ld16(gg + k * THREADS);
-    }
-    if (with_ctrl) {
-      const u32x4* ga = reinterpret_cast<const u32x4*>(p.action + r0 * NA) + tid;
-#pragma unroll
-      for (int k = 0; k < KA; ++k)
-        if (k * THREADS + THREADS <= CA || tid + k * THREADS < CA) ra[k] = ld16(ga + k * THREADS);
-    }
-  };
-
-  long tile = blockIdx.x;
-  if (tile < ntiles) issue_loads(tile);
-  for (; tile < ntiles; tile += gridDim.x) {
+  for (; tile < ntiles; tile += wgs) {
     const long row0 = tile * ROWS;
     {
       u32x4* lq = reinterpret_cast<u32x4*>(sq) + tid;
@@ -549,7 +561,8 @@
       }
     }
     __syncthreads();
-    const long next = tile + gridDim.x;
+    const double prev0 = prev;
+    const long next = tile + wgs;
     if (next < ntiles) issue_loads(next);
 
     if (tid < ROWS) {
@@ -571,7 +584,7 @@
       if (rt == OLY_REWARD_NONE) {
         p.reward[gr] = 0.0f;
       } else {
-        if (gr < p.N) p.reward[gr] = rew_f(p.prev_in[gr]);
+        if (gr < p.N) p.reward[gr] = rew_f(prev0);
         if (gr + p.N < p.R)
           p.reward[gr + p.N] = rew_f(x);
         else
@@ -695,6 +708,12 @@
   const int nq = md->nq, nv = md->nv, n_grf = md->n_grf, n_act = md->n_act, nu = md->nu, n_obs = md->n_obs;
   const DynCarve cv(nq, nv, n_grf, n_act, nu, n_obs);
   const int tid = threadIdx.x, lane = tid & 63;
+  const long ntiles = p.tile0;
+  if ((int)blockIdx.x >= p.tile_wgs) {
+    il_step_tile<ROWS, THREADS, DynDims, OBS64, CTRL64>(p, ntiles);
+    return;
+  }
+  const int wgs = p.tile_wgs;
   double* sq = reinterpret_cast<double*>(lds);
   float* sa = reinterpret_cast<float*>(lds + cv.a);
   unsigned* eo = reinterpret_cast<unsigned*>(lds + cv.eo);
@@ -721,12 +740,10 @@
     co[e] = k < 0 ? -1 : (((r * n_act + k) << 8) | j);
   }
   for (int j = tid; j < nu; j += THREADS) {
-    const int k = md->ctrl_src[j];
-    const int kk = k < 0 ? 0 : k;
-    t_act[j] = md->act_mean[kk];
-    t_act[nu + j] = md->act_delta[kk];
-    t_act[2 * nu + j] = md->ctrl_lo[kk];
-    t_act[3 * nu + j] = md->ctrl_hi[kk];
+    t_act[j] = md->act_tab[j];
+    t_act[nu + j] = md->act_tab[OLY_MAX_ACT + j];
+    t_act[2 * nu + j] = md->act_tab[2 * OLY_MAX_ACT + j];
+    t_act[3 * nu + j] = md->act_tab[3 * OLY_MAX_ACT + j];
   }
   const int nf = md->n_fall;
   const int rt = md->reward_type;
@@ -796,15 +813,14 @@
       la[g] = ld16(reinterpret_cast<const u32x4*>(p.action + row0 * n_act) + g);
   };
 
-  const long ntiles = p.tile0;
   long tile = blockIdx.x;
   if (tile < ntiles) issue_loads(tile);
   __syncthreads();
-  for (; tile < ntiles; tile += gridDim.x) {
+  for (; tile < ntiles; tile += wgs) {
     const long row0 = tile * ROWS;
     land(row0);
     __syncthreads();
-    const long next = tile + gridDim.x;
+    const long next = tile + wgs;
     if (next < ntiles) issue_loads(next);
 
     if (tid < ROWS) {
@@ -912,7 +928,7 @@
 using AtlasFullDims = StaticDims<31, 31, 0, 25, 25, 60>;
 using TalosFullDims = StaticDims<30, 30, 0, 24, 24, 58>;
 
-template <int ROWS, class D>
+template <int ROWS, class D, int TH = THREADS>
 int launch_generic(oly_ctx* ctx, IlArgs a, long tile0, int out_flags, hipStream_t s) {
   const IlDev& h = ctx->il_host;
   Carve<ROWS, D> cv(h.nq, h.nv, h.n_grf, h.n_act, h.nu, h.n_obs);
@@ -920,11 +936,11 @@
   if (tiles <= 0) return OLY_OK;
   if (tiles > 0x7fffffffL) OLY_FAIL(ctx, OLY_EINVAL, "oly_il_step: too many rows");
   a.tile0 = tile0;
-  dim3 grid((unsigned)tiles), block(THREADS);
+  dim3 grid((unsigned)tiles), block(TH);
   const bool o64 = out_flags & OLY_OUT_OBS_F64, c64 = out_flags & OLY_OUT_CTRL_F64;
 #define OLY_K1(O, C_)                                                                       \
   do {                                                                                      \
-    auto k = il_step_kernel<ROWS, D, O, C_>;                                                \
+    auto k = il_step_kernel<ROWS, TH, D, O, C_>;                                             \
     if (cv.total > 48 * 1024)                                                               \
       OLY_HIP(ctx, hipFuncSetAttribute(reinterpret_cast<const void*>(k),                    \
                                        hipFuncAttributeMaxDynamicSharedMemorySize, cv.total)); \
@@ -939,11 +955,33 @@
   return OLY_OK;
 }
 
+constexpr int SMALL_ROWS = 16;
+inline int small_rows(const oly_ctx* ctx, long R, int big_rows) {
+  static const int env = [] { const char* e = getenv("OLY_K1_SMALL_ROWS"); return e ? atoi(e) : -1; }();
+  if (env == 0) return 0;
+  const int cus = ctx->num_cu > 0 ? ctx->num_cu : 256;
+  if ((R + big_rows - 1) / big_rows >= cus) return 0;
+  int rows = env == 16 || env == 32 || env == 64 ? env : SMALL_ROWS;
+  if (ctx->il_max_wg > 0) {
+    while (rows < 64 && (R + rows - 1) / rows > ctx->il_max_wg) rows *= 2;
+    if ((R + rows - 1) / rows > ctx->il_max_wg) return 0;
+  }
+  return rows;
+}
+template <class D>
+int launch_small(oly_ctx* ctx, int rows, IlArgs a, int out_flags, hipStream_t s) {
+  if (rows == 64) return launch_generic<64, D, 256>(ctx, a, 0, out_flags, s);
+  if (rows == 32) return launch_generic<32, D, 128>(ctx, a, 0, out_flags, s);
+  return launch_generic<16, D, 64>(ctx, a, 0, out_flags, s);
+}
+
 template <int ROWS, class D>
-int launch_fast(oly_ctx* ctx, IlArgs a, int out_flags, int wg_per_cu, hipStream_t s) {
+int launch_fast(oly_ctx* ctx, IlArgs a, int out_flags, int wg_per_cu, hipStream_t s, bool allow_small = true) {
+  if (const int sr = allow_small ? small_rows(ctx, a.R, ROWS) : 0) return launch_small<D>(ctx, sr, a, out_flags, s);
   const long nfull = a.R / ROWS;
+  const bool ragged = nfull * ROWS < a.R;
   if (nfull > 0) {
-    const int lds = ROWS * (D::nq + D::nv + D::n_grf) * 8 + ROWS * D::n_act * 4 + 4 * D::nu * 8;
+    int lds = ROWS * (D::nq + D::nv + D::n_grf) * 8 + ROWS * D::n_act * 4 + 4 * D::nu * 8;
     int per_cu = (160 * 1024) / lds;
     if (per_cu > 8) per_cu = 8;
     if (wg_per_cu > 0) per_cu = wg_per_cu;
@@ -951,6 +989,12 @@
     if (want > nfull) want = nfull;
     IlArgs b = a;
     b.tile0 = nfull;
+    b.tile_wgs = (int)want;
+    if (ragged) {
+      const Carve<ROWS, D> cv(D::nq, D::nv, D::n_grf, D::n_act, D::nu, D::n_obs);
+      if (cv.total > lds) lds = cv.total;
+      ++want;
+    }
     dim3 grid((unsigned)want), block(THREADS);
     const bool o64 = out_flags & OLY_OUT_OBS_F64, c64 = out_flags & OLY_OUT_CTRL_F64;
 #define OLY_K1T(O, C_)                                                                      \
@@ -967,32 +1011,38 @@
     else OLY_K1T(false, false);
 #undef OLY_K1T
     OLY_LAUNCH_CHECK(ctx, "il_tile_kernel");
-  }
-  if (nfull * ROWS < a.R) return launch_generic<ROWS, D>(ctx, a, nfull, out_flags, s);
-  return OLY_OK;
+    return OLY_OK;
+  }
+  return launch_generic<ROWS, D>(ctx, a, 0, out_flags, s);
 }
 
 int launch_dyn(oly_ctx* ctx, IlArgs a, int out_flags, hipStream_t s) {
   const IlDev& h = ctx->il_host;
   const DynCarve cv(h.nq, h.nv, h.n_grf, h.n_act, h.nu, h.n_obs);
-  const long nfull = (a.fast && cv.total <= 150 * 1024) ? a.R / DYN_ROWS : 0;
+  if (a.fast)
+    if (const int sr = small_rows(ctx, a.R, DYN_ROWS)) return launch_small<DynDims>(ctx, sr, a, out_flags, s);
+  const Carve<DYN_ROWS, DynDims> gcv(h.nq, h.nv, h.n_grf, h.n_act, h.nu, h.n_obs);
+  const int lds = cv.total > gcv.total ? cv.total : gcv.total;
+  const long nfull = (a.fast && lds <= 150 * 1024) ? a.R / DYN_ROWS : 0;
   if (nfull > 0) {
-    int per_cu = (160 * 1024) / cv.total;
+    int per_cu = (160 * 1024) / lds;
     if (per_cu > 4) per_cu = 4;
     if (per_cu < 1) per_cu = 1;
     long want = (long)ctx->num_cu * per_cu;
     if (want > nfull) want = nfull;
     IlArgs b = a;
     b.tile0 = nfull;
+    b.tile_wgs = (int)want;
+    if (nfull * DYN_ROWS < a.R) ++want;
     dim3 grid((unsigned)want), block(THREADS);
     const bool o64 = out_flags & OLY_OUT_OBS_F64, c64 = out_flags & OLY_OUT_CTRL_F64;
 #define OLY_K1D(O, C_)                                                                      \
   do {                                                                                      \
     auto k = il_dyn_tile_kernel<O, C_>;                                                     \
-    if (cv.total > 48 * 1024)                                                               \
+    if (lds > 48 * 1024)                                                                    \
       OLY_HIP(ctx, hipFuncSetAttribute(reinterpret_cast<const void*>(k),                    \
-                                       hipFuncAttributeMaxDynamicSharedMemorySize, cv.total)); \
-    hipLaunchKernelGGL(k, grid, block, cv.total, s, b);                                     \
+                                       hipFuncAttributeMaxDynamicSharedMemorySize, lds));   \
+    hipLaunchKernelGGL(k, grid, block, lds, s, b);                                          \
   } while (0)
     if (o64 && c64) OLY_K1D(true, true);
     else if (o64) OLY_K1D(true, false);
@@ -1000,9 +1050,9 @@
     else OLY_K1D(false, false);
 #undef OLY_K1D
     OLY_LAUNCH_CHECK(ctx, "il_dyn_tile_kernel");
-  }
-  if (nfull * DYN_ROWS < a.R) return launch_generic<DYN_ROWS, DynDims>(ctx, a, nfull, out_flags, s);
-  return OLY_OK;
+    return OLY_OK;
+  }
+  return launch_generic<DYN_ROWS, DynDims>(ctx, a, 0, out_flags, s);
 }
 
 inline bool al16(const void* p) { return (reinterpret_cast<uintptr_t>(p) & 15) == 0; }
@@ -1064,6 +1114,11 @@
     h.act_mean[k] = m->act_mean[k]; h.act_delta[k] = m->act_delta[k];
     h.ctrl_lo[k] = m->ctrl_lo[k]; h.ctrl_hi[k] = m->ctrl_hi[k];
   }
+  for (int j = 0; j < m->nu; ++j) {
+    const int kk = h.ctrl_src[j] < 0 ? 0 : h.ctrl_src[j];
+    h.act_tab[j] = h.act_mean[kk]; h.act_tab[OLY_MAX_ACT + j] = h.act_delta[kk];
+    h.act_tab[2 * OLY_MAX_ACT + j] = h.ctrl_lo[kk]; h.act_tab[3 * OLY_MAX_ACT + j] = h.ctrl_hi[kk];
+  }
   OLY_HIP(ctx, hipSetDevice(ctx->device));
   OLY_HIP(ctx, hipMemcpy(ctx->il_dev, &h, sizeof(h), hipMemcpyHostToDevice));
   ctx->il_ok = true;
@@ -1094,12 +1149,14 @@
   if (ctrl && !action) OLY_FAIL(ctx, OLY_EINVAL, "oly_il_step: ctrl requested without action");
   IlArgs a;
   a.md = ctx->il_dev; a.R = (long)T * N; a.N = N; a.qpos = qpos; a.qvel = qvel; a.action = action;
-  a.grf = h.n_grf ? grf_mean : nullptr; a.prev_in = prev_in; a.prev_out = prev_out; a.obs = obs;
+  a.grf = h.n_grf ? grf_mean : nullptr;
+  a.prev_in = h.reward_type != OLY_REWARD_NONE ? prev_in : nullptr;
+   a.prev_out = prev_out; a.obs = obs;
   a.reward = reward; a.absorbing = absorbing; a.fall_code = fall_code; a.ctrl = ctrl;
   a.fast = al16(qpos) && al16(qvel) && al16(action) && al16(grf_mean) && al16(obs) && al16(ctrl) &&
            ((reinterpret_cast<uintptr_t>(absorbing) & 3) == 0) &&
            ((reinterpret_cast<uintptr_t>(fall_code) & 3) == 0);
-  a.tile0 = 0;
+  a.tile0 = 0; a.tile_wgs = 0;
   auto shape = [&](int nq, int na, int no, int ng = 0) {
     return h.nq == nq && h.nv == nq && h.n_grf == ng && h.n_act == na && h.nu == na && h.n_obs == no &&
            h.n_pos == nq && h.n_vel == nq && h.n_drop == 2;
@@ -1109,9 +1166,9 @@
   static const int rows_env = [] { const char* e = getenv("OLY_K1_ROWS"); return e ? atoi(e) : 0; }();
 #define OLY_K1_FAST(DIMS, DEFROWS)                                                              \
   do {                                                                                          \
-    const int rows = rows_env ? rows_env : DEFROWS;                                             \
-    if (rows == 64) return launch_fast<64, DIMS>(ctx, a, out_flags, wg_env, oly_s(stream));     \
-    return launch_fast<128, DIMS>(ctx, a, out_flags, wg_env, oly_s(stream));                    \
+    const int rows = rows_env ? rows_env : DEFROWS;    \
+    if (rows == 64) return launch_fast<64, DIMS>(ctx, a, out_flags, wg_env, oly_s(stream), !rows_env); \
+    return launch_fast<128, DIMS>(ctx, a, out_flags, wg_env, oly_s(stream), !rows_env);         \
   } while (0)
   if (fast_ok && shape(17, 11, 32)) OLY_K1_FAST(H1Dims, 128);
   if (fast_ok && shape(16, 10, 30)) OLY_K1_FAST(AtlasDims, 128);
diff --git a/olympics-mujoco_amd/csrc/oly_common.h b/olympics-mujoco_amd/csrc/oly_common.h
--- a/olympics-mujoco_amd/csrc/oly_common.h
+++ b/olympics-mujoco_amd/csrc/oly_common.h
@@ -18,6 +18,7 @@
   double fall_lo[OLY_MAX_FALL], fall_hi[OLY_MAX_FALL];
   short ctrl_src[OLY_MAX_ACT];
   double act_mean[OLY_MAX_ACT], act_delta[OLY_MAX_ACT], ctrl_lo[OLY_MAX_ACT], ctrl_hi[OLY_MAX_ACT];
+  double act_tab[4 * OLY_MAX_ACT];
 };
 
 struct A3Dev {
@@ -72,6 +73,7 @@
   unsigned discfit_attr_done = 0;
   unsigned gail_attr_done = 0;
   int num_cu;
+  int il_max_wg = 0;
 };
 
 #define OLY_FAIL(ctx, code, ...)                                \
```

Measured after the change: 12.43 billion env-steps/s, median of 2. Within noise of the previous version (+0.1%).
